# Xiugapurin/Etude

Measured on AMD Instinct MI355X. Metric: audio-sec/s transcribed + decoder tokens/s, 3-min clip batch, higher is better.
Workload: dtype f16

## Files before the change

### etude_amd/_lib.py

```python
from __future__ import annotations

import ctypes as C
import os
from pathlib import Path

import torch

LIB_PATH = Path(os.environ["ETD_LIB_PATH"]) if os.environ.get("ETD_LIB_PATH") else Path(__file__).resolve().parent / "libetude_hip.so"

c_int_p = C.POINTER(C.c_int)
c_i32_p = C.POINTER(C.c_int32)
c_i64_p = C.POINTER(C.c_int64)
c_f32_p = C.POINTER(C.c_float)


class _SizedCfg(C.Structure):

    def __init__(self, *a, **k):
        super().__init__(*a, **k)
        self.struct_bytes = C.sizeof(type(self))


class ExtCfg(_SizedCfg):
    _fields_ = [("struct_bytes", C.c_int)] + [(n, C.c_int) for n in ("n_margin", "n_frame", "n_bin", "cnn_channel", "cnn_kernel", "hid_dim", "pf_dim",
# ... 24 lines not shown
    _fields_ = [("struct_bytes", C.c_int), ("kernel", C.c_int), ("epi", C.c_int)] + [(n, C.c_int) for n in ("M", "N", "K", "ldx", "ldy")] + \
               [("X", C.c_void_p), ("x_elems", C.c_longlong), ("W", C.c_void_p), ("bias", C.c_void_p), ("x_bound", C.c_float),
                ("ln_g", C.c_void_p), ("ln_b", C.c_void_p), ("ln_eps", C.c_float), ("Y", C.c_void_p), ("y_elems", C.c_longlong),
                ("add", C.c_void_p), ("hin", C.c_void_p), ("hout", C.c_void_p), ("h_elems", C.c_longlong),
                ("pos", C.c_void_p), ("slot", C.c_void_p), ("active", C.c_void_p)] + [(n, C.c_int) for n in ("n_heads", "max_ctx", "n_slots", "rope_rows")] + \
               [("rope_cos", C.c_void_p), ("rope_sin", C.c_void_p), ("Q", C.c_void_p), ("q_elems", C.c_longlong), ("Kc", C.c_void_p), ("Vc", C.c_void_p), ("kv_elems", C.c_longlong)]


G3_KERNEL_AUTO, G3_KERNEL_TILE, G3_KERNEL_SMALL = 0, 1, 2
G3_EPI = {"bias": 0, "gelu": 1, "resid": 2, "logits": 3, "qkv": 4, "relu": 6}


class Job(C.Structure):
    _fields_ = [("x_ids", C.c_void_p), ("x_offsets", C.c_void_p), ("n_bars", C.c_int), ("attrs4", C.c_void_p), ("ready", C.c_void_p)]


class ScoreJob(C.Structure):
    _fields_ = [("x_ids", C.c_void_p), ("x_offsets", C.c_void_p), ("n_bars", C.c_int), ("attrs4", C.c_void_p),
                ("y_ids", C.c_void_p), ("y_offsets", C.c_void_p), ("n_y_bars", C.c_int)]


class SchedCfg(_SizedCfg):
    _fields_ = [("struct_bytes", C.c_int)] + [(n, C.c_int) for n in ("bar_bos_id", "bar_eos_id", "n_ctx_pairs", "max_position_embeddings", "max_output_tokens",
                                       "max_bar_token_limit")] + [("context_overlap_ratio", C.c_float)] + \
               [(n, C.c_int) for n in ("force_bar_tokens", "max_streams", "max_prefill_rows", "steps_per_poll")] + \
               [("temperature", C.c_float), ("top_p", C.c_float), ("seed", C.c_ulonglong), ("job_key_offset", C.c_int), ("job_key_stride", C.c_int)]


class TempoRegion(C.Structure):
    _fields_ = [("bpm", C.c_double), ("time_sig", C.c_int), ("start", C.c_double), ("downbeats", C.c_void_p), ("n_downbeats", C.c_int)]


class TokEvent(C.Structure):
    _fields_ = [("type", C.c_int32), ("value", C.c_int32)]


class Note(C.Structure):
    _fields_ = [("onset", C.c_double), ("offset", C.c_double), ("pitch", C.c_int32), ("velocity", C.c_int32)]


ABI_VERSION = 3

SIGNATURES = {
    "etd_version": (C.c_int, []),
    "etd_last_error": (C.c_char_p, []),
    "etd_build_id": (C.c_char_p, []),
    "etd_extractor_operand_type": (C.c_int, []),
    "etd_decoder_operand_type": (C.c_int, []),
    "etd_has_experiments": (C.c_int, []),
    "etd_prof_enable": (C.c_int, [C.c_int]),
    "etd_prof_reset": (C.c_int, []),
    "etd_prof_collect": (C.c_int, []),
    "etd_prof_count": (C.c_int, []),
    "etd_prof_entry": (C.c_int, [C.c_int, C.c_char_p, C.c_int, C.POINTER(C.c_double), C.POINTER(C.c_longlong),
                                 C.POINTER(C.c_double), C.POINTER(C.c_double)]),
    "etd_debug_boundary_cost": (C.c_int, [C.c_int, C.c_int, C.c_int, C.c_void_p, C.POINTER(C.c_double), C.POINTER(C.c_double)]),
    "etd_debug_linear": (C.c_int, [C.c_int, C.c_int, C.c_int, C.c_int, C.c_void_p, C.POINTER(C.c_double)]),
    "etd_debug_kernel_loop": (C.c_int, [C.c_int, C.c_int, C.c_void_p]),
    "etd_debug_g3_bounds": (C.c_int, [C.c_void_p, C.c_void_p, C.c_int, C.c_int, C.c_void_p, C.c_void_p, C.c_float, C.c_void_p, C.c_void_p]),
    "etd_debug_gemm3": (C.c_int, [C.c_void_p, C.c_int, C.c_int, C.c_void_p, C.c_void_p, C.c_int, C.c_float, C.c_int, C.c_void_p, C.c_void_p, C.c_void_p, C.c_void_p]),
    "etd_debug_gemm3_case": (C.c_int, [C.POINTER(G3Case), C.c_void_p]),
    "etd_debug_ln_rows_f32": (C.c_int, [C.c_void_p, C.c_int, C.c_int, C.c_void_p, C.c_void_p, C.c_void_p, C.c_void_p, C.c_float, C.c_void_p, C.c_void_p, C.c_void_p]),
    "etd_debug_g3_pack": (C.c_int, [C.c_void_p, C.c_int, C.c_int, C.c_void_p, C.c_longlong, C.POINTER(C.c_longlong), C.POINTER(C.c_int32)]),
    "etd_debug_attn3": (C.c_int, [C.c_void_p, C.c_void_p, C.c_void_p, C.c_void_p, C.c_int, C.c_int, C.c_int, C.c_int, C.c_float, C.c_float, C.c_float, C.c_int, C.c_void_p, C.c_void_p]),
    "etd_debug_empty_launch": (C.c_int, [C.c_int, C.c_int, C.c_int, C.c_void_p, C.c_void_p]),
    "etd_frontend_create": (C.c_int, [C.c_int, C.c_int, C.c_int, C.c_int, C.c_int, C.c_int, C.c_void_p, C.c_int, C.c_int,
                                      C.c_void_p, C.c_int, C.c_void_p, C.c_void_p, C.c_void_p, C.c_float, C.POINTER(C.c_void_p)]),
    "etd_frontend_destroy": (None, [C.c_void_p]),
    "etd_frontend_set_pad_mode": (C.c_int, [C.c_void_p, C.c_int]),
    "etd_rms_frames": (C.c_int, [C.c_void_p, C.c_longlong, C.c_int, C.c_int, C.c_void_p, C.c_longlong, C.c_void_p]),
    "etd_frontend_resampled_len": (C.c_longlong, [C.c_void_p, C.c_longlong]),
    "etd_frontend_num_frames": (C.c_longlong, [C.c_void_p, C.c_longlong]),
    "etd_frontend_run": (C.c_int, [C.c_void_p, C.c_void_p, C.c_int, C.c_longlong, C.c_void_p, C.c_void_p, C.c_longlong,
                                   C.POINTER(C.c_longlong), C.c_void_p]),
    "etd_extractor_create": (C.c_int, [C.POINTER(ExtCfg), C.POINTER(C.c_char_p), C.POINTER(C.c_void_p), c_i64_p, C.c_int,
                                       C.POINTER(C.c_void_p)]),
    "etd_extractor_destroy": (None, [C.c_void_p]),
    "etd_transcript": (C.c_int, [C.c_void_p, C.c_void_p, C.c_longlong] + [C.c_void_p] * 8 + [C.c_void_p]),
    "etd_transcript_windows": (C.c_int, [C.c_void_p, C.c_void_p, C.c_int] + [C.c_void_p] * 8 + [C.c_void_p]),
    "etd_extractor_debug_vel_logits": (C.c_int, [C.c_void_p, C.c_void_p]),
    "etd_extractor_debug_tap": (C.c_int, [C.c_void_p, C.c_int, C.c_void_p]),
    "etd_extractor_window_flops": (C.c_double, [C.c_void_p]),
    "etd_mpe2note": (C.c_int, [C.c_void_p, C.c_void_p, C.c_void_p, C.c_void_p, C.c_longlong, C.c_int, C.c_float, C.c_float,
                               C.c_float, C.c_int, C.c_int, C.c_int, C.POINTER(Note), C.c_longlong, C.POINTER(C.c_longlong)]),
    "etd_mpe2note_modes": (C.c_int, [C.c_void_p, C.c_void_p, C.c_void_p, C.c_void_p, C.c_longlong, C.c_int, C.c_float, C.c_float,
                                     C.c_float, C.c_int, C.c_int, C.c_int, C.c_int, C.c_int, C.POINTER(Note), C.c_longlong, C.POINTER(C.c_longlong)]),
    "etd_mpe2note_dev_create": (C.c_int, [C.c_int, C.POINTER(C.c_void_p)]),
    "etd_mpe2note_dev_destroy": (None, [C.c_void_p]),
    "etd_mpe2note_dev": (C.c_int, [C.c_void_p, C.c_void_p, C.c_void_p, C.c_void_p, C.c_void_p, C.c_longlong, C.c_float, C.c_float, C.c_float,
                                   C.c_int, C.c_int, C.c_int, C.POINTER(Note), C.c_longlong, C.POINTER(C.c_longlong), C.c_void_p]),
    "etd_mpe2note_dev_modes": (C.c_int, [C.c_void_p, C.c_void_p, C.c_void_p, C.c_void_p, C.c_void_p, C.c_longlong, C.c_float, C.c_float, C.c_float,
                                         C.c_int, C.c_int, C.c_int, C.c_int, C.c_int, C.POINTER(Note), C.c_longlong, C.POINTER(C.c_longlong), C.c_void_p]),
    "etd_tok_create": (C.c_int, [C.c_void_p, C.c_int, C.POINTER(C.c_void_p)]),
    "etd_tok_destroy": (None, [C.c_void_p]),
    "etd_tok_num_measures": (C.c_int, [C.c_void_p]),
    "etd_tok_measures": (C.c_int, [C.c_void_p, C.c_void_p, C.c_void_p, C.c_void_p, C.c_void_p]),
    "etd_tok_encode": (C.c_int, [C.c_void_p, C.c_void_p, C.c_longlong, C.c_int, C.c_void_p, C.c_longlong, C.POINTER(C.c_longlong)]),
    "etd_tok_split_bars": (C.c_int, [C.c_void_p, C.c_longlong, C.c_int, C.c_int, C.c_void_p, C.c_longlong, C.c_void_p, C.c_longlong,
                                     C.POINTER(C.c_longlong)]),
    "etd_tok_decode": (C.c_int, [C.c_void_p, C.c_void_p, C.c_longlong, C.c_void_p, C.c_longlong, C.c_void_p, C.c_longlong,
                                 C.POINTER(C.c_longlong)]),
    "etd_midi_write": (C.c_int, [C.c_void_p, C.c_longlong, C.c_char_p]),
    "etd_decoder_create": (C.c_int, [C.POINTER(DecCfg), C.POINTER(C.c_char_p), C.POINTER(C.c_void_p), c_i64_p, C.c_int,
                                     C.POINTER(C.c_void_p)]),
    "etd_decoder_destroy": (None, [C.c_void_p]),
    "etd_decoder_clone": (C.c_int, [C.c_void_p, C.POINTER(C.c_void_p)]),
    "etd_decoder_set_sampling": (C.c_int, [C.c_void_p, C.c_float, C.c_float, C.c_ulonglong, C.c_void_p]),
    "etd_decoder_set_keys": (C.c_int, [C.c_void_p, C.c_int, C.c_void_p, C.c_void_p]),
    "etd_decoder_begin_bar": (C.c_int, [C.c_void_p, C.c_int, C.c_void_p, C.c_void_p, C.c_void_p, C.c_int, C.c_void_p, C.c_int,
                                        C.c_int, C.c_void_p]),
    "etd_decoder_begin_bars": (C.c_int, [C.c_void_p, C.c_int] + [C.c_void_p] * 8 + [C.c_void_p]),
    "etd_decoder_step": (C.c_int, [C.c_void_p, C.c_void_p, C.c_int, C.c_int, C.c_void_p]),
    "etd_decoder_poll": (C.c_int, [C.c_void_p, C.c_void_p, C.c_int, C.c_void_p, C.c_void_p, C.c_void_p]),
    "etd_decoder_read_tokens": (C.c_int, [C.c_void_p, C.c_int, C.c_void_p, C.c_int, c_int_p, C.c_void_p]),
    "etd_decoder_read_many": (C.c_int, [C.c_void_p, C.c_int, C.c_void_p, C.c_void_p, C.c_int, C.c_void_p, C.c_void_p]),
    "etd_decoder_run_jobs": (C.c_int, [C.c_void_p, C.POINTER(SchedCfg), C.POINTER(Job), C.c_int, C.c_void_p, C.c_longlong, C.c_void_p,
                                       C.POINTER(C.c_longlong), C.c_void_p]),
    "etd_debug_assemble_prompt": (C.c_int, [C.POINTER(SchedCfg), C.c_int, C.c_void_p, C.c_void_p, C.c_void_p, C.c_void_p, C.c_void_p, C.c_void_p,
                                            C.c_int, C.c_void_p, C.c_void_p, C.c_void_p, C.c_void_p, C.c_int, c_int_p]),
    "etd_decoder_generate_bar": (C.c_int, [C.c_void_p, C.c_int, C.c_void_p, C.c_void_p, C.c_void_p, C.c_int, C.c_void_p,
                                           C.c_int, C.c_int, C.c_void_p, c_int_p, C.c_void_p]),
    "etd_decoder_prefill_logits": (C.c_int, [C.c_void_p, C.c_int, C.c_void_p, C.c_void_p, C.c_void_p, C.c_int, C.c_void_p,
                                             C.c_void_p]),
    "etd_decoder_score": (C.c_int, [C.c_void_p, C.c_int] + [C.c_void_p] * 11 + [C.c_void_p]),
    "etd_decoder_score_jobs": (C.c_int, [C.c_void_p, C.POINTER(SchedCfg), C.POINTER(ScoreJob), C.c_int, C.c_void_p, C.c_void_p, C.c_void_p, C.c_void_p]),
    "etd_debug_assemble_scored": (C.c_int, [C.POINTER(SchedCfg), C.c_int, C.c_void_p, C.c_void_p, C.c_void_p, C.c_void_p, C.c_void_p, C.c_void_p,
                                            C.c_int, C.c_void_p, C.c_int, C.c_void_p, C.c_void_p, C.c_void_p, C.c_void_p, C.c_void_p, C.c_int, c_int_p]),
    "etd_decoder_step_bytes": (C.c_double, [C.c_void_p, C.c_int, C.c_int]),
    "etd_decoder_stats": (C.c_int, [C.c_void_p, C.POINTER(C.c_double), C.c_int, C.c_void_p]),
    "etd_decoder_stats_reset": (C.c_int, [C.c_void_p, C.c_void_p]),
    "etd_decoder_stamp": (C.c_int, [C.c_void_p, C.c_int, C.c_int, C.c_void_p]),
    "etd_decoder_stamp_log": (C.c_int, [C.c_void_p, C.c_void_p, C.c_longlong, C.POINTER(C.c_longlong), C.c_void_p]),
    "etd_debug_decoder_force_pair": (C.c_int, [C.c_void_p, C.c_int]),
    "etd_debug_decoder_step_logits": (C.c_int, [C.c_void_p, C.c_int, C.c_void_p, C.c_int, C.c_void_p]),
    "etd_debug_decoder_checksum": (C.c_int, [C.c_void_p, C.POINTER(C.c_ulonglong), C.c_int, C.c_void_p]),
    "etd_debug_decoder_kv_rowsums": (C.c_int, [C.c_void_p, C.c_void_p, C.c_longlong, C.c_void_p]),
    "etd_debug_decoder_trace_begin": (C.c_int, [C.c_void_p, C.c_int, C.c_void_p]),
    "etd_debug_decoder_trace_slabs": (C.c_int, [C.c_void_p, C.c_void_p, C.c_longlong, C.c_int, C.c_void_p]),
    "etd_debug_decoder_trace_lanes": (C.c_int, [C.c_void_p, C.c_void_p, C.c_longlong, C.c_int, C.c_void_p]),
    "etd_debug_decoder_trace_q": (C.c_int, [C.c_void_p, C.c_void_p, C.c_longlong, C.c_int, C.c_void_p]),
    "etd_debug_decoder_peek_kv": (C.c_int, [C.c_void_p, C.c_int, C.c_int, C.c_int, C.c_int, C.c_void_p, C.c_void_p, C.c_void_p]),
    "etd_beat_create": (C.c_int, [C.POINTER(BeatCfg), C.POINTER(C.c_char_p), C.POINTER(C.c_void_p), c_i64_p, C.c_int, C.POINTER(C.c_void_p)]),
    "etd_beat_destroy": (None, [C.c_void_p]),
    "etd_beat_forward": (C.c_int, [C.c_void_p, C.c_void_p, C.c_int, c_i64_p, C.c_void_p, C.c_void_p, C.c_void_p]),
    "etd_beat_flops": (C.c_double, [C.c_void_p, C.c_longlong]),
    "etd_beat_debug_taps": (C.c_int, [C.c_void_p, C.c_void_p, C.c_void_p]),
    "etd_dbn_describe": (C.c_int, [C.POINTER(DbnCfg), C.c_int, C.c_void_p, C.c_int, c_int_p, c_int_p, c_int_p, C.c_void_p, C.c_void_p]),
    "etd_dbn_workspace_bytes": (C.c_longlong, [C.POINTER(DbnCfg), C.c_longlong, C.c_int]),
    "etd_dbn_create": (C.c_int, [C.POINTER(DbnCfg), C.POINTER(C.c_void_p)]),
    "etd_dbn_destroy": (None, [C.c_void_p]),
    "etd_dbn_track": (C.c_int, [C.c_void_p, C.c_void_p, C.c_int, C.c_int, c_i64_p, C.c_void_p, C.c_longlong, C.c_void_p, C.c_void_p, C.c_void_p, C.c_longlong,
                                C.c_void_p, C.c_void_p, C.POINTER(C.c_longlong), C.c_void_p]),
    "etd_dbn_debug_viterbi": (C.c_int, [C.c_void_p, C.c_int, C.c_void_p, C.c_longlong, C.c_void_p, C.POINTER(C.c_double)]),
    "etd_debug_decoder_trace_read": (C.c_int, [C.c_void_p, C.c_void_p, C.c_longlong, C.c_int, C.POINTER(C.c_int), C.c_void_p]),
}

_lib = None


class EtudeHipError(RuntimeError):
    pass


def lib() -> C.CDLL:
    global _lib
    if _lib is None:
        if not LIB_PATH.exists():
            raise EtudeHipError(f"{LIB_PATH} not found: build it with `python -m etude_amd.build` "
                                "(hipcc --offload-arch=gfx950); etude_amd has no CPU fallback")
        l = C.CDLL(str(LIB_PATH))
        for name, (res, args) in SIGNATURES.items():
            if os.environ.get("ETD_PARTIAL") and not hasattr(l, name):
                continue
            fn = getattr(l, name)
            fn.restype = res
            fn.argtypes = args
        if l.etd_version() != ABI_VERSION:
            raise EtudeHipError(f"{LIB_PATH} speaks ABI version {l.etd_version()}, this binding {ABI_VERSION}; rebuild with `python -m etude_amd.build`")
        if not os.environ.get("ETD_PARTIAL") and not os.environ.get("ETD_ALLOW_STALE_LIB"):
            from .build import src_hash
            have, want = (l.etd_build_id() or b"").decode(), src_hash()
            if have != want:
                raise EtudeHipError(f"{LIB_PATH} is stale: built from sources {have}, the tree is {want}; rebuild with `python -m etude_amd.build`")
        _lib = l
    return _lib


def check(rc: int, what: str = "") -> None:
    if rc != 0:
        msg = lib().etd_last_error()
        raise EtudeHipError(f"{what} failed (rc={rc}): {msg.decode() if msg else ''}")


def weights_arrays(state: dict):
    import numpy as np
    names = list(state.keys())
    arrs = [np.ascontiguousarray(np.asarray(state[k], dtype=np.float32)) for k in names]
    c_names = (C.c_char_p * len(names))(*[k.encode() for k in names])
    c_ptrs = (C.c_void_p * len(names))(*[a.ctypes.data for a in arrs])
    c_num = (C.c_int64 * len(names))(*[a.size for a in arrs])
    return c_names, c_ptrs, c_num, len(names), arrs


def prof_enable(on: bool) -> None:
    lib().etd_prof_enable(1 if on else 0)


def prof_reset() -> None:
    lib().etd_prof_reset()


def prof_report() -> dict:
    l = lib()
    l.etd_prof_collect()
    out = {}
    for i in range(l.etd_prof_count()):
        name = C.create_string_buffer(64)
        ms, n, fl, by = C.c_double(), C.c_longlong(), C.c_double(), C.c_double()
        check(l.etd_prof_entry(i, name, 64, C.byref(ms), C.byref(n), C.byref(fl), C.byref(by)), "etd_prof_entry")
        out[name.value.decode()] = dict(ms=ms.value, launches=n.value, flops=fl.value, bytes=by.value)
    return out
```

### etude_amd/csrc/api_dec.hip

```cpp
#include <algorithm>
#include <atomic>
#include <chrono>
#include <cmath>
#include <cstdlib>
#include <cstring>
#include <map>
#include <string>
#include <mutex>
#include <vector>

#include "../../include/etude_hip_debug.h"
#include "dec_kernels.h"
#include "gemm3.h"
#include "ext_kernels.h"
#include "dec_score.h"
#include "prof.h"

namespace {

inline uint16_t f2bf_h(float f) { return ETD_DEC_IS_F16 ? f32_to_f16_bits(f) : f32_to_bf16_bits(f); }

struct Lin { void* W = nullptr; float* b = nullptr; int N = 0, Npad = 0, K = 0;
             void* Wf = nullptr;
             G3Lin g3; };
// ... 177 lines not shown
  const Layer& w = d->layers[l];
  return launch_ln_rows(h, M, d->H, w.ln1g, w.ln1b, w.ln2g, w.ln2b, d->cfg.layer_norm_eps, d->X1b, d->X2b, st);
}
static int layer_dattn(etd_dec* d, int l, const DecRows& rows, int M, d16* Ob, int ldob, hipStream_t st) {
  DAttnArgs at = attn_args(d, l, rows, M); at.O = d->AO; at.Ob = Ob; at.ldob = ldob;
  if (rows.slot == d->row_slot) { attn_step_pairs(d, &at); attn_stamp(d, l, &at); }
  return launch_dattn(at, d->bf16w, st);
}
static int step_qkv_up(etd_dec* d, int l, const float* X, const DecRows& rows, int M, hipStream_t st) {
  DGemmArgs q = qkv_args(d, l, X, rows, M); q.Xb = d->X1b; q.Y = d->qkv_raw; q.ldy = 3 * d->H;
  DGemmArgs up = lin_args(d->layers[l].up, X, d->H, M); up.Xb = d->X2b; up.Y = d->M1; up.Yb = d->Xcat; up.ldy = d->I + d->H;
  return launch_dstep_qkv_up(q, up, st);
}
static int resid_ln(etd_dec* d, int l, int nslab, const float* hin, float* hout, int M, const NextLn& nx, hipStream_t st) {
  return launch_resid_ln_rows(d->Pk, nslab, d->layers[l].cat.b, nullptr, hin, hout, M, d->H, nx.g1, nx.b1, nx.g2, nx.b2, d->cfg.layer_norm_eps, nx.x1, nx.x2, st);
}
static int down_splitk(etd_dec* d, int l, const float* hin, float* hout, int M, const NextLn& nx, hipStream_t st) {
  DGemmArgs dn = lin_args(d->layers[l].cat, d->M1, d->I + d->H, M); dn.Xb = d->Xcat; dn.hin = hin; dn.hout = hout; dn.k_splits = DS_K_SPLITS; dn.Y = d->Pk; dn.ldy = d->H;
  ETD_TRY(launch_dgemm(dn, DEPI_PARTIAL, true, st));
  return resid_ln(d, l, DS_K_SPLITS, hin, hout, M, nx, st);
}
static int linear16(const Lin& w, const d16* X, int M, const DGemmArgs& dec, int epi, hipStream_t st) {
  LinArgs a = {};
  a.X = (const e16*)X; a.ldx = w.K; a.W = (const e16*)w.Wf;
  a.bias = w.b; a.M = M; a.N = w.N; a.K = w.K; a.vt_block = -1; a.dec = dec;
  return launch_linear_dec(a, epi, st);
}

static int gemm3_auto(const DGemmArgs& a, int epi, hipStream_t st) { return gemm3_s_takes(a, epi) ? launch_gemm3_s(a, epi, st) : launch_gemm3(a, epi, st); }
static int x3_last_rows(etd_dec* d, const LastOnly& lo, const float* hin, float* hout, hipStream_t st) {
  const int n = lo.n, l = d->L - 1, H = d->H; const Layer& w = d->layers[l];
  ETD_TRY(launch_gather_rows(hin, lo.idx, n, H, d->hlast, st)); ETD_TRY(launch_gather_rows(d->Q, lo.idx, n, H, d->t_q, st));
  DAttnArgs at = attn_args(d, l, lo.rows, n); at.Q = d->t_q; at.O = d->t_ao; at.bytes_hint = 0;
  ETD_TRY(launch_dattn(at, false, st));
  DGemmArgs de = lin_args(w.dense, d->t_ao, H, n); de.Y = d->t_do; de.ldy = H;
  ETD_TRY(launch_dgemm(de, DEPI_BIAS, false, st));
  DGemmArgs up = lin_args(w.up, d->hlast, H, n); up.Y = d->t_m1; up.ldy = d->I; up.ln_g = w.ln2g; up.ln_b = w.ln2b; up.ln_eps = d->cfg.layer_norm_eps;
  ETD_TRY(launch_dgemm(up, DEPI_GELU, false, st));
  DGemmArgs dn = lin_args(w.down, d->t_m1, d->I, n); dn.add = d->t_do; dn.hin = d->hlast; dn.hout = hout;
  return launch_dgemm(dn, DEPI_RESID, false, st);
}
static int x3_layer_rest(etd_dec* d, int l, const DecRows& rows, int M, const PrefillInfo* pf, const float* hin, float* hout, hipStream_t st) {
  const Layer& w = d->layers[l]; const int H = d->H;
  if (pf) {
    Attn3Args t = {};
    t.Q = d->Q; t.ldq = H; t.K = (const float*)kv_layer(d, d->Kc, l); t.V = (const float*)kv_layer(d, d->Vc, l); t.O = d->AO; t.ldo = H; t.n_seq = pf->n; t.n_heads = d->nh;
    t.seq_row0 = pf->seq_row0; t.seq_len = pf->seq_len; t.row_slot = rows.slot; t.slot_stride = d->slot_stride; t.max_ctx = d->ctx; t.max_len = pf->max_len;
    t.scale = 0.125f; t.q_log2 = w.q_log2; t.k_log2 = w.k_log2; t.v_log2 = w.v_log2; t.flops_hint = pf->attn_flops;
    ETD_TRY(launch_attn3(t, st));
  } else {
    DAttnArgs at = attn_args(d, l, rows, M);
    at.O = d->AO; attn_stamp(d, l, &at);
    if (rows.slot == d->row_slot) attn_step_pairs(d, &at);
    ETD_TRY(launch_dattn(at, false, st));
  }
  DGemmArgs de = lin_args(w.dense, d->AO, H, M); de.Y = d->DO; de.ldy = H;
  ETD_TRY(gemm3_auto(de, DEPI_BIAS, st));
  DGemmArgs up = lin_args(w.up, d->X2f, H, M); up.Y = d->M1; up.ldy = d->I;
  ETD_TRY(gemm3_auto(up, DEPI_GELU, st));
  DGemmArgs dn = lin_args(w.down, d->M1, d->I, M); dn.add = d->DO; dn.hin = hin; dn.hout = hout;
  return gemm3_auto(dn, DEPI_RESID, st);
}
static int forward_x3(etd_dec* d, int M, const DecRows& rows, const PrefillInfo* pf, const LastOnly* lo, hipStream_t st, float** hfinal, bool* compact) {
  const bool tail = lo && pf && lo->n >= 1 && lo->n < G3_MIN_ROWS && lo->n <= d->S;
  float* hin = d->h; float* hout = d->h2;
  for (int l = 0; l < d->L; ++l) {
    const Layer& w = d->layers[l];
    ETD_TRY(launch_ln_rows_f32(hin, M, d->H, w.ln1g, w.ln1b, w.ln2g, w.ln2b, d->cfg.layer_norm_eps, d->X1f, d->X2f, st));
    ETD_TRY(gemm3_auto(qkv_args(d, l, d->X1f, rows, M), DEPI_QKV, st));
    ETD_TRY(tail && l == d->L - 1 ? x3_last_rows(d, *lo, hin, hout, st) : x3_layer_rest(d, l, rows, M, pf, hin, hout, st));
    std::swap(hin, hout);
  }
  *hfinal = hin; if (tail) *compact = true;
  return ETD_OK;
}

static int forward_plain(etd_dec* d, int M, const DecRows& rows, bool act16, hipStream_t st, float** hfinal) {
  float* hin = d->h; float* hout = d->h2; const float eps = d->cfg.layer_norm_eps;
  for (int l = 0; l < d->L; ++l) {
    const Layer& w = d->layers[l];
    if (act16) ETD_TRY(ln_rows16(d, l, hin, M, st));
    DGemmArgs q = qkv_args(d, l, hin, rows, M); q.Y = d->qkv_raw; q.ldy = 3 * d->H;
    if (act16) q.Xb = d->X1b; else { q.ln_g = w.ln1g; q.ln_b = w.ln1b; q.ln_eps = eps; }
    ETD_TRY(launch_dgemm(q, DEPI_QKV, d->bf16w, st));
    ETD_TRY(layer_dattn(d, l, rows, M, act16 ? d->AOb : nullptr, 0, st));
    DGemmArgs de = lin_args(w.dense, d->AO, d->H, M); de.Y = d->DO; de.ldy = d->H; if (act16) de.Xb = d->AOb;
    ETD_TRY(launch_dgemm(de, DEPI_BIAS, d->bf16w, st));
    DGemmArgs up = lin_args(w.up, hin, d->H, M); up.Y = d->M1; up.ldy = d->I;
    if (act16) { up.Xb = d->X2b; up.Yb = d->M1b; } else { up.ln_g = w.ln2g; up.ln_b = w.ln2b; up.ln_eps = eps; }
    ETD_TRY(launch_dgemm(up, DEPI_GELU, d->bf16w, st));
    DGemmArgs dn = lin_args(w.down, d->M1, d->I, M); dn.add = d->DO; dn.hin = hin; dn.hout = hout; if (act16) dn.Xb = d->M1b;
    ETD_TRY(launch_dgemm(dn, DEPI_RESID, d->bf16w, st));
    std::swap(hin, hout);
  }
  *hfinal = hin;
  return ETD_OK;
}

static int trace_qkv_up(etd_dec* d, int l, int M, hipStream_t st) {
  if (!d->trace) return ETD_OK;
  ETD_TRY(trace_rows(d, d->Q, d->H, d->H, 1, 0, M, l * ETD_TRACE_LAYER * M, st));
  if (l == 0) HIP_TRY(hipMemcpyAsync(d->trace_q, d->Q, (size_t)M * d->H * 4, hipMemcpyDeviceToDevice, st));
  ETD_TRY(trace_rows(d, d->Xcat, (d->I + d->H) / 2, d->I / 2, 1, 0, M, l * ETD_TRACE_LAYER * M + M, st));
  if (d->nh == 8) {
    hipLaunchKernelGGL(k_trace_kv, dim3(M, 8), dim3(64), 0, st, (const unsigned*)kv_layer(d, d->Kc, l), (const unsigned*)kv_layer(d, d->Vc, l), d->slot_stride / 2, d->ctx,
                       d->row_slot, d->row_pos, M, d->trace, d->trace_step, d->trace_cap, trace_wps(d, M), l * ETD_TRACE_LAYER * M + 17 * M);
    HIP_TRY(hipGetLastError());
  }
  return ETD_OK;
}
static int skinny_attn_down(etd_dec* d, int l, const DecRows& rows, int M, const float* hin, float* hout, hipStream_t st) {
  const Layer& w = d->layers[l]; const NextLn nx = next_ln(d, l);
  const int ksd = d->I / 512;
  DAttnArgs at = attn_args(d, l, rows, M);
  attn_step_pairs(d, &at); attn_stamp(d, l, &at); at.pair = d->step_pair ? 1 : 0;
  at.dense_w = (const d16*)w.dense_hw; at.dense_out = d->Pk + (size_t)ksd * M * d->H; at.dbg = (d->trace && l == 0) ? d->trace_dbg : nullptr;
  DGemmArgs dn = lin_args(w.cat, nullptr, d->I + d->H, M); dn.Xb = d->Xcat; dn.k_splits = ksd; dn.Y = d->Pk; dn.ldy = d->H;
  if (rowfin_on() && ksd + d->nh == 12 && M <= DS_STEP_MAX_ROWS) {
    DRowFin fin = {};
    fin.cnt = d->row_cnt + (size_t)l * DS_STEP_MAX_ROWS; fin.target = d->nh + 16 * ksd; fin.P = d->Pk; fin.nslab = 12;
    fin.bias = w.cat.b; fin.hin = hin; fin.hout = hout; fin.eps = d->cfg.layer_norm_eps;
    fin.g1 = nx.g1; fin.b1 = nx.b1; fin.g2 = nx.g2; fin.b2 = nx.b2; fin.x1 = nx.x1; fin.x2 = nx.x2;
    return launch_dstep_attn_down(at, dn, &fin, st);
  }
  ETD_TRY(launch_dstep_attn_down(at, dn, nullptr, st));
  if (d->trace && ksd + d->nh == 12) ETD_TRY(trace_rows(d, d->Pk, d->H, d->H, 12, (long long)M * d->H, M, l * ETD_TRACE_LAYER * M + 2 * M, st));
  if (d->trace && l == 0 && ksd + d->nh == 12) HIP_TRY(hipMemcpyAsync(d->trace_pk, d->Pk, (size_t)12 * M * d->H * 4, hipMemcpyDeviceToDevice, st));
  ETD_TRY(resid_ln(d, l, ksd + d->nh, hin, hout, M, nx, st));
  if (d->trace) {
    ETD_TRY(trace_rows(d, hout, d->H, d->H, 1, 0, M, l * ETD_TRACE_LAYER * M + 14 * M, st));
    if (nx.x1) {
      ETD_TRY(trace_rows(d, d->X1b, d->H / 2, d->H / 2, 1, 0, M, l * ETD_TRACE_LAYER * M + 15 * M, st));
      ETD_TRY(trace_rows(d, d->X2b, d->H / 2, d->H / 2, 1, 0, M, l * ETD_TRACE_LAYER * M + 16 * M, st));
    }
  }
  return ETD_OK;
}
static int forward_skinny16(etd_dec* d, int M, const DecRows& rows, bool ln0_done, hipStream_t st, float** hfinal) {
  const bool attn_down = rows.slot == d->row_slot && d->H == 512 && d->nh == 8 && d->I % 512 == 0 && d->I / 512 + d->nh <= 12 && d->layers[0].dense_hw &&
                         d->ctx >= 256 && !getenv("ETD_NO_ATTN_DOWN");
  float* hin = d->h; float* hout = d->h2;
  if (!ln0_done) ETD_TRY(ln_rows16(d, 0, hin, M, st));
  for (int l = 0; l < d->L; ++l) {
    ETD_TRY(step_qkv_up(d, l, hin, rows, M, st));
    ETD_TRY(trace_qkv_up(d, l, M, st));
    if (attn_down) ETD_TRY(skinny_attn_down(d, l, rows, M, hin, hout, st));
    else { ETD_TRY(layer_dattn(d, l, rows, M, d->Xcat + d->I, d->I + d->H, st)); ETD_TRY(down_splitk(d, l, hin, hout, M, next_ln(d, l), st)); }
    std::swap(hin, hout);
  }
  *hfinal = hin;
  return ETD_OK;
}

static int prefill16_qkv(etd_dec* d, int l, const float* hin, const DecRows& rows, int M, bool mfma_attn, hipStream_t st) {
  const Layer& w = d->layers[l];
  DGemmArgs q = qkv_args(d, l, hin, rows, M); q.Xb = d->X1b; q.Y = d->qkv_raw; q.ldy = 3 * d->H;
  if (mfma_attn) q.Qb = d->Qb;
  static const bool pqkv_on = !getenv("ETD_NO_PQKV");
  if (!(mfma_attn && pqkv_on && M >= 49152 && d->H == 512 && d->nh == 8 && w.qkv.N == 1536)) return linear16(w.qkv, d->X1b, M, q, DEPI_QKV, st);
  PQkvArgs pa = {};
  pa.X = d->X1b; pa.ldx = d->H; pa.Wf = (const d16*)w.qkv.Wf; pa.bias = w.qkv.b; pa.M = M; pa.N = w.qkv.N; pa.rows = rows;
  pa.rope_cos = d->rope_cos; pa.rope_sin = d->rope_sin; pa.Qb = d->Qb; pa.Kc = (d16*)q.Kc; pa.Vc = (d16*)q.Vc; pa.slot_stride = d->slot_stride; pa.max_ctx = d->ctx; pa.n_heads = d->nh;
  return launch_pqkv(pa, st);
}
static int prefill16_layer_rest(etd_dec* d, int l, const DecRows& rows, int M, const PrefillInfo* pf, bool fmlp, const float* hin, float* hout, hipStream_t st) {
  const Layer& w = d->layers[l];
  if (pf) {
    PAttnArgs t = {};
    t.Q = d->Qb; t.ldq = d->H; t.Kc = (const d16*)kv_layer(d, d->Kc, l); t.Vc = (const d16*)kv_layer(d, d->Vc, l); t.slot_stride = d->slot_stride; t.max_ctx = d->ctx; t.n_heads = d->nh;
    t.O = d->Xcat + d->I; t.ldo = d->I + d->H; t.seq_row0 = pf->seq_row0; t.seq_len = pf->seq_len; t.row_slot = rows.slot;
    t.n_seq = pf->n; t.max_len = pf->max_len; t.scale_log2e = 0.125f * 1.4426950408889634f; t.flops_hint = pf->attn_flops;
    ETD_TRY(launch_pattn(t, st));
  } else ETD_TRY(layer_dattn(d, l, rows, M, d->Xcat + d->I, d->I + d->H, st));
  if (fmlp) {
    const NextLn nx = next_ln(d, l); DMlpArgs ma = {};
    ma.X2 = d->X2b; ma.AO = d->Xcat + d->I; ma.ldao = d->I + d->H; ma.hin = hin; ma.hout = hout; ma.Wm = (const d16*)w.mlp_frag;
    ma.b_up = w.up.b; ma.b_cat = w.cat.b; ma.eps = d->cfg.layer_norm_eps; ma.M = M;
    ma.g1 = nx.g1; ma.b1 = nx.b1; ma.g2 = nx.g2; ma.b2 = nx.b2; ma.nx1 = nx.x1; ma.nx2 = nx.x2;
    return launch_dmlp_fused(ma, st);
  }
  DGemmArgs up = {}; up.Yb = d->Xcat; up.ldy = d->I + d->H;
  ETD_TRY(linear16(w.up, d->X2b, M, up, DEPI_GELU, st));
  DGemmArgs dn = {}; dn.N = d->H; dn.hin = hin; dn.hout = hout;
  return linear16(w.cat, d->Xcat, M, dn, DEPI_RESID, st);
}
static int prefill16_last_rows(etd_dec* d, const LastOnly& lo, const float* hin, float* hout, hipStream_t st) {
  const int n = lo.n, l = d->L - 1;
  ETD_TRY(launch_gather_rows(hin, lo.idx, n, d->H, d->hlast, st));
  ETD_TRY(ln_rows16(d, l, d->hlast, n, st));
  ETD_TRY(step_qkv_up(d, l, d->hlast, lo.rows, n, st));
  DAttnArgs at = attn_args(d, l, lo.rows, n); at.O = d->AO; at.Ob = d->Xcat + d->I; at.ldob = d->I + d->H; at.bytes_hint = 0;
  ETD_TRY(launch_dattn(at, d->bf16w, st));
  return down_splitk(d, l, d->hlast, hout, n, NextLn{}, st);
}
static int forward_prefill16(etd_dec* d, int M, const DecRows& rows, const PrefillInfo* pf, const LastOnly* lo, hipStream_t st, float** hfinal, bool* compact) {
  const bool fmlp = d->layers[0].mlp_frag && d->H == 512 && d->I == 2048 && fused_pmlp_on();
  const bool tail = lo && pf && lo->n > 1 && lo->n <= DS_STEP_MAX_ROWS && step_shape(d) && !getenv("ETD_NO_LAST_ONLY");
  float* hin = d->h; float* hout = d->h2;
  for (int l = 0; l < d->L; ++l) {
    if (l == 0 || !fmlp) ETD_TRY(ln_rows16(d, l, hin, M, st));
    ETD_TRY(prefill16_qkv(d, l, hin, rows, M, pf != nullptr, st));
    ETD_TRY(tail && l == d->L - 1 ? prefill16_last_rows(d, *lo, hin, hout, st) : prefill16_layer_rest(d, l, rows, M, pf, fmlp, hin, hout, st));
    std::swap(hin, hout);
  }
  *hfinal = hin; if (tail) *compact = true;
  return ETD_OK;
}

static int forward_rows(etd_dec* d, int M, const DecRows& rows, const PrefillInfo* pf, const LastOnly* lo, hipStream_t st, float** hfinal, bool* compact) {
  if (compact) *compact = false; else lo = nullptr;
  const Layer& w0 = d->layers[0];
  if (!d->bf16w && M >= G3_MIN_ROWS && d->X1f && w0.qkv.g3.Wp && w0.down.g3.Wp && g3_enabled()) return forward_x3(d, M, rows, pf, lo, st, hfinal, compact);
  const bool act16 = d->bf16w && M > 1;
  if (act16 && M > DS_MAX_ROWS && w0.qkv.Wf && w0.up.Wf && w0.cat.Wf) return forward_prefill16(d, M, rows, pf, lo, st, hfinal, compact);
  if (act16 && ksplit_fits(d)) return forward_skinny16(d, M, rows, false, st, hfinal);
  return forward_plain(d, M, rows, act16, st, hfinal);
}

int head_logits(etd_dec* d, const float* X, int n, float* logits, hipStream_t st) {
  const bool g3 = !d->bf16w && n >= G3_MIN_ROWS && d->X1f && d->head.g3.Wp && g3_enabled();
  if (g3) ETD_TRY(launch_ln_rows_f32(X, n, d->H, d->lnfg, d->lnfb, nullptr, nullptr, d->cfg.layer_norm_eps, d->X1f, nullptr, st));
  DGemmArgs lm = lin_args(d->head, g3 ? d->X1f : X, d->H, n);
  lm.bias = nullptr; lm.Y = logits; lm.ldy = d->V;
  if (g3) return launch_gemm3(lm, DEPI_LOGITS, st);
  lm.ln_g = d->lnfg; lm.ln_b = d->lnfb; lm.ln_eps = d->cfg.layer_norm_eps;
  return launch_dgemm(lm, DEPI_LOGITS, d->bf16w, st);
}

int check_slot(etd_dec* d, int slot) {
  if (!d || slot < 0 || slot >= d->S) ETD_FAIL(ETD_EINVAL, "decoder: bad slot %d", slot);
  return ETD_OK;
}

__global__ void k_init_slots(const int* __restrict__ init, int n, int* tgt_attrs, int* cur_tok, int* len, int* done, int* n_out, int* eos, int* limit) {
  const int i = blockIdx.x * blockDim.x + threadIdx.x;
  if (i >= n) return;
  const int* p = init + i * 7;
  const int s = p[0];
  tgt_attrs[4 * s] = p[1]; tgt_attrs[4 * s + 1] = p[2]; tgt_attrs[4 * s + 2] = p[3]; tgt_attrs[4 * s + 3] = p[4];
  cur_tok[s] = 0; len[s] = 0; done[s] = 0; n_out[s] = 0; eos[s] = p[5]; limit[s] = p[6];
}

__global__ __launch_bounds__(128) void k_slot_proj(const int* __restrict__ init, const float* __restrict__ attr_tab, int n_bins, int H, float* proj) {
  const int* p = init + blockIdx.x * 7;
  const int s = p[0];
  for (int k = threadIdx.x * 4; k < H; k += 128 * 4) {
    f32x4 t[4];
#pragma unroll
    for (int a = 0; a < 4; ++a) t[a] = *reinterpret_cast<const f32x4*>(attr_tab + (long long)(a * n_bins + p[1 + a]) * H + k);
    f32x4 o;
#pragma unroll
    for (int c = 0; c < 4; ++c) o[c] = ((t[0][c] + t[1][c]) + t[2][c]) + t[3][c];
    *reinterpret_cast<f32x4*>(proj + (long long)s * H + k) = o;
  }
}

struct Staged { int Mtot; const int *ids, *cls, *attrs, *row_slot, *row_pos, *row_active, *last_idx, *last_slot, *last_pos, *last_active, *init, *row_seq, *seq_row0, *seq_len; };

int stage_and_forward(etd_dec* d, int n, const int32_t* slots, const int32_t* T, const int32_t* ids, const int32_t* cls,
                      const int32_t* attrs4, const int32_t* init7 , Staged* sg, float** hfinal, hipStream_t st, bool* last_only = nullptr) {
  if (!d || n < 1 || n > d->S || !slots || !T || !ids || !cls || !attrs4) ETD_FAIL(ETD_EINVAL, "prefill: bad arguments");
  long long Mtot = 0;
  std::vector<char> seen((size_t)d->S, 0);
  for (int i = 0; i < n; ++i) {
    ETD_TRY(check_slot(d, slots[i]));
    if (T[i] <= 0 || T[i] > d->ctx) ETD_FAIL(ETD_EINVAL, "prefill: prompt %d has T=%d (max_ctx=%d)", i, T[i], d->ctx);
    if (seen[slots[i]]) ETD_FAIL(ETD_EINVAL, "prefill: slot %d listed twice", slots[i]);
    seen[slots[i]] = 1;
    Mtot += T[i];
  }
  if (Mtot > d->Mcap) ETD_FAIL(ETD_EINVAL, "prefill: %lld prompt rows exceed max_prefill_rows=%d", Mtot, d->Mcap);
  const int M = (int)Mtot;
  for (int i = 0; i < M; ++i) {
    if (ids[i] < 0 || ids[i] >= d->V || cls[i] < 0 || cls[i] >= d->cfg.num_classes) ETD_FAIL(ETD_EINVAL, "prefill: token/class id out of range at row %d", i);
    for (int k = 0; k < 4; ++k) if (attrs4[(size_t)k * M + i] < 0 || attrs4[(size_t)k * M + i] >= d->cfg.num_attribute_bins) ETD_FAIL(ETD_EINVAL, "prefill: attribute bin out of range at row %d", i);
  }
  const size_t sv_ints = (size_t)10 * M + 13 * n;
  int* svp;
  const bool pinned = d->pin_stage && sv_ints <= d->pin_stage_ints;
  if (pinned) {
    HIP_TRY(hipEventSynchronize(d->pin_stage_evt));
    svp = d->pin_stage;
  } else {
    d->stage.resize(sv_ints);
    svp = d->stage.data();
  }
  memcpy(svp, ids, (size_t)M * 4);
  memcpy(svp + M, cls, (size_t)M * 4);
  memcpy(svp + 2 * (size_t)M, attrs4, (size_t)4 * M * 4);
  int* rs = svp + 6 * (size_t)M; int* rp = rs + M; int* ra = rp + M;
  int* li = ra + M; int* ls = li + n; int* lp = ls + n; int* la = lp + n; int* in7 = la + n;
  int* rq = in7 + 7 * n; int* sr0 = rq + M; int* sln = sr0 + n;
  int row = 0, max_len = 0; double kvb = 0, aflops = 0;
  for (int i = 0; i < n; ++i) {
    sr0[i] = row; sln[i] = T[i]; if (T[i] > max_len) max_len = T[i];
    aflops += 0.5 * 256.0 * d->nh * (double)T[i] * T[i];
    for (int t = 0; t < T[i]; ++t, ++row) { rs[row] = slots[i]; rp[row] = t; ra[row] = 1; rq[row] = i; }
    li[i] = row - 1; ls[i] = slots[i]; lp[i] = T[i] - 1; la[i] = 1;
    d->host_len[slots[i]] = T[i];
    kvb += (double)T[i] * d->nh * 64 * (2.0 * (d->bf16w ? 2 : 4) + 4 + 4);
  }
  if (init7) memcpy(in7, init7, (size_t)7 * n * 4); else memset(in7, 0, (size_t)7 * n * 4);
  d->attn_bytes_hint = kvb;
  HIP_TRY(hipMemcpyAsync(d->ids, svp, sv_ints * 4, hipMemcpyHostToDevice, st));
  if (pinned) HIP_TRY(hipEventRecord(d->pin_stage_evt, st));
  d->host_n_out_valid = false;
  const int* b = d->ids;
  *sg = Staged{M, b, b + M, b + 2 * (size_t)M, b + 6 * (size_t)M, b + 7 * (size_t)M, b + 8 * (size_t)M, b + 9 * (size_t)M, b + 9 * (size_t)M + n,
               b + 9 * (size_t)M + 2 * n, b + 9 * (size_t)M + 3 * n, b + 9 * (size_t)M + 4 * n,
               b + 9 * (size_t)M + 11 * n, b + 10 * (size_t)M + 11 * n, b + 10 * (size_t)M + 12 * n};
  if (init7) {
    hipLaunchKernelGGL(k_init_slots, dim3((n + 63) / 64), dim3(64), 0, st, sg->init, n, d->tgt_attrs, d->cur_tok, d->len, d->done, d->n_out, d->eos, d->limit);
    HIP_TRY(hipGetLastError());
    hipLaunchKernelGGL(k_slot_proj, dim3(n), dim3(128), 0, st, sg->init, d->attr_tab, d->cfg.num_attribute_bins, d->H, d->tgt_proj);
    HIP_TRY(hipGetLastError());
  }
  DEmbedArgs e = {};
  e.ids = sg->ids; e.cls = sg->cls; e.attrs = sg->attrs; e.M = M; e.H = d->H; e.n_bins = d->cfg.num_attribute_bins;
  e.word = d->word; e.cls_emb = d->cls_emb; e.attr_tab = d->attr_tab; e.h = d->h;
  e.rows = DecRows{sg->row_slot, sg->row_pos, sg->row_active, sg->row_seq};
  ETD_TRY(launch_dembed(e, st));
  PrefillInfo pf{n, sg->seq_row0, sg->seq_len, max_len, aflops};
  const bool can_mfma_attn = (d->bf16w ? d->Qb != nullptr : d->X1f != nullptr) && !ETD_XENV("ETD_NO_MFMA_PREFILL_ATTN");
  LastOnly lo{n, sg->last_idx, DecRows{sg->last_slot, sg->last_pos, sg->last_active}};
  return forward_rows(d, M, e.rows, can_mfma_attn ? &pf : nullptr, &lo, st, hfinal, last_only);
}

int alloc_workspaces(etd_dec* d) {
  const int H = d->H;
  DevPool& P = d->pool;
  d->slot_stride = (long long)d->nh * d->ctx * 64;
  d->layer_stride = d->slot_stride * d->S;
  const size_t kv_elems = (size_t)d->layer_stride * d->L;
  if (d->bf16w) { uint16_t *k, *v; ETD_TRY(P.alloc(&k, kv_elems, true)); ETD_TRY(P.alloc(&v, kv_elems, true)); d->Kc = k; d->Vc = v; }
  else { float *k, *v; ETD_TRY(P.alloc(&k, kv_elems, true)); ETD_TRY(P.alloc(&v, kv_elems, true)); d->Kc = k; d->Vc = v; }
  const size_t M = d->Mcap;
  const size_t Mf = d->bf16w ? (size_t)(d->S > 1 ? d->S : 1) : M;
  ETD_TRY(P.alloc(&d->h, M * H)); ETD_TRY(P.alloc(&d->h2, M * H));
  ETD_TRY(P.alloc(&d->Q, M * H)); ETD_TRY(P.alloc(&d->AO, M * H)); ETD_TRY(P.alloc(&d->DO, M * H));
  ETD_TRY(P.alloc(&d->M1, Mf * d->I)); ETD_TRY(P.alloc(&d->logits, (size_t)d->Mmax * d->V));
  ETD_TRY(P.alloc(&d->qkv_raw, (size_t)3 * H)); ETD_TRY(P.alloc(&d->hlast, (size_t)d->S * H));
  if (d->bf16w) {
    ETD_TRY(P.alloc(&d->X1b, M * H)); ETD_TRY(P.alloc(&d->X2b, M * H)); ETD_TRY(P.alloc(&d->AOb, M * H));
    ETD_TRY(P.alloc(&d->M1b, M * d->I));
    ETD_TRY(P.alloc(&d->Pk, (size_t)12 * DS_STEP_MAX_ROWS * H));
    ETD_TRY(P.alloc(&d->row_cnt, (size_t)d->L * DS_STEP_MAX_ROWS, true));
    ETD_TRY(P.alloc(&d->Xcat, M * (d->I + H)));
    ETD_TRY(P.alloc(&d->Qb, M * H));
  }
  if (!d->bf16w) {
    ETD_TRY(P.alloc(&d->X1f, M * H)); ETD_TRY(P.alloc(&d->X2f, M * H));
    const size_t Sr = d->S > 1 ? d->S : 1;
    ETD_TRY(P.alloc(&d->t_q, Sr * H)); ETD_TRY(P.alloc(&d->t_ao, Sr * H)); ETD_TRY(P.alloc(&d->t_do, Sr * H)); ETD_TRY(P.alloc(&d->t_m1, Sr * d->I));
  }
// ... 658 lines not shown
  const bool full = logits_dev != nullptr;
  std::vector<int32_t> slots(S), a4c, up;
  for (int i = 0; i < S; ++i) slots[i] = i;
  long long r0 = 0;
  for (int i0 = 0; i0 < n;) {
    int k = 0; long long Mc = 0;
    while (i0 + k < n && k < S && (k == 0 || Mc + T[i0 + k] <= rowcap)) Mc += T[i0 + k++];
    const int mc = (int)Mc;
    a4c.resize((size_t)4 * mc);
    for (int a = 0; a < 4; ++a) memcpy(a4c.data() + (size_t)a * mc, attrs4 + a * M + r0, (size_t)mc * 4);
    up.assign(labels + r0, labels + r0 + mc);
    for (int r = 0; r < mc; ++r) if (full || labels[r0 + r] != ETD_IGNORE_LABEL) up.push_back(r);
    const int nl = (int)up.size() - mc;
    const int nblk = (nl + hb - 1) / hb;
    up.resize((size_t)mc + (size_t)nblk * hb, 0);
    HIP_TRY(hipMemcpyAsync(lab_dev, up.data(), (size_t)mc * 4, hipMemcpyHostToDevice, st));
    if (nblk) HIP_TRY(hipMemcpyAsync(idx_dev, up.data() + mc, (size_t)nblk * hb * 4, hipMemcpyHostToDevice, st));
    up.clear();
    for (int i = 0, row = 0; i < k; ++i) { up.push_back(row); row += T[i0 + i]; }
    up.insert(up.end(), T + i0, T + i0 + k);
    HIP_TRY(hipMemcpyAsync(r0_dev, up.data(), (size_t)k * 4, hipMemcpyHostToDevice, st));
    HIP_TRY(hipMemcpyAsync(len_dev, up.data() + k, (size_t)k * 4, hipMemcpyHostToDevice, st));
    if (row_lp || row_argmax) {
      HIP_TRY(hipMemsetAsync(lp_dev, 0, (size_t)mc * 4, st));
      HIP_TRY(hipMemsetAsync(am_dev, 0xff, (size_t)mc * 4, st));
    }
    Staged sg; float* hf = nullptr;
    ETD_TRY(stage_and_forward(d, k, slots.data(), T + i0, ids + r0, cls + r0, a4c.data(), nullptr, &sg, &hf, st));
    for (int b = 0; b < nblk; ++b) {
      const int nb = std::min(hb, nl - b * hb);
      ETD_TRY(launch_gather_rows(hf, idx_dev + (size_t)b * hb, hb, d->H, d->sc_x, st));
      ETD_TRY(head_logits(d, d->sc_x, hb, d->logits, st));
      ETD_TRY(launch_row_logprob(d->logits, d->V, d->V, nb, idx_dev + (size_t)b * hb, lab_dev, lp_dev, lse_dev, am_dev, st));
      if (full) HIP_TRY(hipMemcpyAsync(logits_dev + (size_t)(r0 + (long long)b * hb) * d->V, d->logits, (size_t)nb * d->V * 4, hipMemcpyDeviceToDevice, st));
    }
    ETD_TRY(launch_seq_reduce(r0_dev, len_dev, k, lab_dev, lp_dev, am_dev, d->sc_d, tok_dev, hit_dev, st));
    HIP_TRY(hipMemcpyAsync(seq_logprob + i0, d->sc_d, (size_t)k * sizeof(double), hipMemcpyDeviceToHost, st));
    HIP_TRY(hipMemcpyAsync(seq_tokens + i0, tok_dev, (size_t)k * 4, hipMemcpyDeviceToHost, st));
    HIP_TRY(hipMemcpyAsync(seq_hits + i0, hit_dev, (size_t)k * 4, hipMemcpyDeviceToHost, st));
    if (row_lp) HIP_TRY(hipMemcpyAsync(row_lp + r0, lp_dev, (size_t)mc * 4, hipMemcpyDeviceToHost, st));
    if (row_argmax) HIP_TRY(hipMemcpyAsync(row_argmax + r0, am_dev, (size_t)mc * 4, hipMemcpyDeviceToHost, st));
    HIP_TRY(hipStreamSynchronize(st));
    i0 += k; r0 += mc;
  }
  return ETD_OK;
}

__global__ void k_sum_words(const unsigned* __restrict__ p, long long n, unsigned long long* out) {
  unsigned long long s = 0;
  for (long long i = blockIdx.x * (long long)blockDim.x + threadIdx.x; i < n; i += (long long)gridDim.x * blockDim.x) s += (unsigned long long)p[i] * (unsigned long long)((i & 1023) + 1);
  for (int o = 32; o > 0; o >>= 1) s += __shfl_xor(s, o, 64);
  if ((threadIdx.x & 63) == 0) atomicAdd(out, s);
}
extern "C" int etd_debug_decoder_checksum(etd_dec* d, unsigned long long* out, int cap, void* stream) {
  hipStream_t st = (hipStream_t)stream;
  if (!d || !out || cap < 1) ETD_FAIL(ETD_EINVAL, "decoder_checksum: bad arguments");
  const size_t first = d->weights_owner ? 0 : d->n_weight_allocs;
  const size_t n = d->pool.ptrs.size() - first;
  unsigned long long* acc = nullptr;
  HIP_TRY(hipMalloc(&acc, 8 * (n + 1)));
  HIP_TRY(hipMemsetAsync(acc, 0, 8 * (n + 1), st));
  for (size_t i = 0; i < n; ++i)
    hipLaunchKernelGGL(k_sum_words, dim3(1024), dim3(256), 0, st, (const unsigned*)d->pool.ptrs[first + i], (long long)(d->pool.bytes[first + i] / 4), acc + 1 + i);
  std::vector<unsigned long long> h(n + 1);
  HIP_TRY(hipMemcpyAsync(h.data(), acc, 8 * (n + 1), hipMemcpyDeviceToHost, st));
  HIP_TRY(hipStreamSynchronize(st));
  (void)hipFree(acc);
  for (size_t i = 1; i <= n; ++i) h[0] += h[i];
  for (int i = 0; i < cap; ++i) out[i] = (size_t)i <= n ? h[i] : 0ull;
  return ETD_OK;
}

__global__ void k_kv_rowsums(const unsigned* __restrict__ K, const unsigned* __restrict__ V, int L, int S, int nh, int ctx, unsigned* out) {
  const long long i = blockIdx.x * (long long)blockDim.x + threadIdx.x;
  if (i >= (long long)L * S * ctx) return;
  const int pos = (int)(i % ctx), slot = (int)((i / ctx) % S), l = (int)(i / ((long long)ctx * S));
  unsigned s = 0;
  for (int hd = 0; hd < nh; ++hd) {
    const long long w0 = ((((long long)l * S + slot) * nh + hd) * ctx + pos) * 32;
    for (int w = 0; w < 32; ++w) s += K[w0 + w] * (unsigned)(w + 1 + 64 * hd) + V[w0 + w] * (unsigned)(w + 33 + 64 * hd);
  }
  out[i] = s;
}
extern "C" int etd_debug_decoder_kv_rowsums(etd_dec* d, unsigned* out_host, long long cap, void* stream) {
  hipStream_t st = (hipStream_t)stream;
  if (!d || !out_host || !d->bf16w) ETD_FAIL(ETD_EINVAL, "kv_rowsums: d16 handles only");
  const long long n = (long long)d->L * d->S * d->ctx;
  if (cap < n) ETD_FAIL(ETD_ENOMEM, "kv_rowsums: need room for %lld words", n);
  unsigned* dev = nullptr;
  HIP_TRY(hipMalloc(&dev, n * 4));
  hipLaunchKernelGGL(k_kv_rowsums, dim3((unsigned)((n + 255) / 256)), dim3(256), 0, st, (const unsigned*)d->Kc, (const unsigned*)d->Vc, d->L, d->S, d->nh, d->ctx, dev);
  HIP_TRY(hipMemcpyAsync(out_host, dev, n * 4, hipMemcpyDeviceToHost, st));
  HIP_TRY(hipStreamSynchronize(st));
  (void)hipFree(dev);
  return ETD_OK;
}

extern "C" int etd_debug_decoder_trace_begin(etd_dec* d, int cap_steps, void* stream) {
  hipStream_t st = (hipStream_t)stream;
  if (!d || cap_steps < 1 || !d->bf16w) ETD_FAIL(ETD_EINVAL, "trace_begin: bad args");
  HIP_TRY(hipStreamSynchronize(st));
  for (auto& kv : d->graphs) (void)hipGraphExecDestroy(kv.second);
  d->graphs.clear();
  if (d->trace) { (void)hipFree(d->trace); d->trace = nullptr; }
  if (d->trace_step) { (void)hipFree(d->trace_step); d->trace_step = nullptr; }
  if (d->trace_pk) { (void)hipFree(d->trace_pk); d->trace_pk = nullptr; }
  if (d->trace_q) { (void)hipFree(d->trace_q); d->trace_q = nullptr; }
  HIP_TRY(hipMalloc(&d->trace_pk, (size_t)12 * d->S * d->H * 4));
  HIP_TRY(hipMalloc(&d->trace_q, (size_t)d->S * d->H * 4));
  if (!d->trace_dbg) HIP_TRY(hipMalloc(&d->trace_dbg, (size_t)d->nh * d->S * 256 * 8 * 4));
  const size_t bytes = (size_t)cap_steps * trace_wps(d, d->S) * 4;
  HIP_TRY(hipMalloc(&d->trace, bytes));
  HIP_TRY(hipMalloc(&d->trace_step, 4));
  HIP_TRY(hipMemsetAsync(d->trace, 0, bytes, st));
  HIP_TRY(hipMemsetAsync(d->trace_step, 0, 4, st));
  HIP_TRY(hipStreamSynchronize(st));
  d->trace_cap = cap_steps;
  return ETD_OK;
}
extern "C" int etd_debug_decoder_trace_slabs(etd_dec* d, float* out_host, long long cap_floats, int n_active, void* stream) {
  hipStream_t st = (hipStream_t)stream;
  if (!d || !d->trace_pk || !out_host || n_active < 1 || n_active > d->S) ETD_FAIL(ETD_EINVAL, "trace_slabs: bad args");
  const long long n = 12LL * n_active * d->H;
  if (cap_floats < n) ETD_FAIL(ETD_ENOMEM, "trace_slabs: need room for %lld floats", n);
  HIP_TRY(hipMemcpyAsync(out_host, d->trace_pk, (size_t)n * 4, hipMemcpyDeviceToHost, st));
  HIP_TRY(hipStreamSynchronize(st));
  return ETD_OK;
}
extern "C" int etd_debug_decoder_trace_lanes(etd_dec* d, float* out_host, long long cap_floats, int n_active, void* stream) {
  hipStream_t st = (hipStream_t)stream;
  const long long n = (long long)(d ? d->nh : 0) * n_active * 256 * 8;
  if (!d || !d->trace_dbg || !out_host || n_active < 1 || n_active > d->S || cap_floats < n) ETD_FAIL(ETD_EINVAL, "trace_lanes: bad args");
  HIP_TRY(hipMemcpyAsync(out_host, d->trace_dbg, (size_t)n * 4, hipMemcpyDeviceToHost, st));
  HIP_TRY(hipStreamSynchronize(st));
  return ETD_OK;
}
extern "C" int etd_debug_decoder_trace_q(etd_dec* d, float* out_host, long long cap_floats, int n_active, void* stream) {
  hipStream_t st = (hipStream_t)stream;
  if (!d || !d->trace_q || !out_host || n_active < 1 || n_active > d->S || cap_floats < (long long)n_active * d->H) ETD_FAIL(ETD_EINVAL, "trace_q: bad args");
  HIP_TRY(hipMemcpyAsync(out_host, d->trace_q, (size_t)n_active * d->H * 4, hipMemcpyDeviceToHost, st));
  HIP_TRY(hipStreamSynchronize(st));
  return ETD_OK;
}
extern "C" int etd_debug_decoder_peek_kv(etd_dec* d, int layer, int slot, int head, int n_pos, unsigned short* k_out, unsigned short* v_out, void* stream) {
  hipStream_t st = (hipStream_t)stream;
  if (!d || !d->bf16w || layer < 0 || layer >= d->L || slot < 0 || slot >= d->S || head < 0 || head >= d->nh || n_pos < 1 || n_pos > d->ctx || !k_out || !v_out)
    ETD_FAIL(ETD_EINVAL, "peek_kv: bad args");
  const size_t off = ((size_t)layer * d->layer_stride + (size_t)slot * d->slot_stride + (size_t)head * d->ctx * 64) * 2;
  HIP_TRY(hipMemcpyAsync(k_out, (const char*)d->Kc + off, (size_t)n_pos * 128, hipMemcpyDeviceToHost, st));
  HIP_TRY(hipMemcpyAsync(v_out, (const char*)d->Vc + off, (size_t)n_pos * 128, hipMemcpyDeviceToHost, st));
  HIP_TRY(hipStreamSynchronize(st));
  return ETD_OK;
}
extern "C" int etd_debug_decoder_trace_read(etd_dec* d, unsigned* out_host, long long cap_words, int n_active, int* steps_done, void* stream) {
  hipStream_t st = (hipStream_t)stream;
  if (!d || !d->trace || !out_host || !steps_done || n_active < 1 || n_active > d->S) ETD_FAIL(ETD_EINVAL, "trace_read: bad args");
  const long long n = (long long)d->trace_cap * trace_wps(d, n_active);
  if (cap_words < n) ETD_FAIL(ETD_ENOMEM, "trace_read: need room for %lld words", n);
  HIP_TRY(hipMemcpyAsync(out_host, d->trace, (size_t)n * 4, hipMemcpyDeviceToHost, st));
  HIP_TRY(hipMemcpyAsync(steps_done, d->trace_step, 4, hipMemcpyDeviceToHost, st));
  HIP_TRY(hipStreamSynchronize(st));
  return ETD_OK;
}

extern "C" double etd_decoder_step_bytes(const etd_dec* d, int n_streams, int ctx) {
  const double esz = d->bf16w ? 2.0 : 4.0;
  double w = 0;
  for (const Layer& l : d->layers) w += ((double)l.qkv.N * l.qkv.K + (double)l.dense.N * l.dense.K + (double)l.up.N * l.up.K + (double)l.down.N * l.down.K) * esz;
  w += (double)d->V * d->H * esz;
  const double kv = (double)n_streams * 2.0 * d->L * (double)(ctx + 1) * d->H * esz;
  return w + kv;
}
```

### etude_amd/csrc/dec_kernels.h

```cpp
#pragma once
#include "common.h"

#ifdef ETD_DEC_BF16
typedef bf16 d16; typedef bf16x8 d16x8; typedef bf16x4 d16x4; typedef bf16x2 d16x2;
#define ETD_MFMA16_DEC "v_mfma_f32_32x32x16_bf16"
#define ETD_DEC_IS_F16 0
#ifdef __HIPCC__
__device__ __forceinline__ d16x4 pack4d(float a, float b, float c, float d) { return pack4(a, b, c, d); }
#endif
#else
typedef f16 d16; typedef f16x8 d16x8; typedef f16x4 d16x4; typedef f16x2 d16x2;
#define ETD_MFMA16_DEC "v_mfma_f32_32x32x16_f16"
#define ETD_DEC_IS_F16 1
#ifdef __HIPCC__
__device__ __forceinline__ d16x4 pack4d(float a, float b, float c, float d) { return pack4h(a, b, c, d); }
#endif
#endif

#define DS_MAX_ROWS 512
#define DS_STEP_MAX_ROWS 2048

struct DecRows {
  const int* slot;
  const int* pos;
  const int* active;
  const int* seq;
};

struct DSampleCfg { float inv_temp; float top_p; unsigned long long seed; };

#define ETD_STAMP_HDR (8 + 2 * 64)
#define ETD_STAMP_LOGCAP 131072

enum { DEPI_BIAS = 0, DEPI_GELU = 1, DEPI_RESID = 2, DEPI_LOGITS = 3, DEPI_QKV = 4, DEPI_PARTIAL = 5, DEPI_RELU = 6  };

struct DGemmArgs {
  const float* X; int ldx;
  const void* W;
  const void* Wf;
  const float* bias;
  int M, N, K;
  int Npad;
  const float* ln_g; const float* ln_b; float ln_eps;
  float* Y; int ldy;
  d16* Yb;
  int k_splits;
  const d16* Xb;
  const float* add; const float* hin; float* hout;
  DecRows rows;
  const float* rope_cos; const float* rope_sin;
  int rot_half;
  float* Q;
  void* Kc; void* Vc;
  long long slot_stride;
  int max_ctx, n_heads;
  d16* Qb;
  const void* Wp; int w_log2;
  int x_log2;
};
int launch_dgemm(const DGemmArgs& a, int epi, bool w_bf16, hipStream_t st);
int launch_dstep_qkv_up(const DGemmArgs& q, const DGemmArgs& up, hipStream_t st);

struct DHeadArgs {
  const float* hfin; int M, H, V, Vpad;
  const float* lnf_g; const float* lnf_b; float eps;
  const d16* Whead;
  int* row_slot; int* row_pos; int* row_active; int* row_sp;
  int* cur_tok; int* len; int* done; int* n_out; int* out_tok; int out_cap; const int* eos; const int* limit;
  const int* tgt_attrs; const float* tgt_proj ; int tgt_cls; int n_bins;
  const float* word; const float* cls_emb; const float* attr_tab;
  const float* g1; const float* b1; const float* g2; const float* b2;
  float* h; d16* x1; d16* x2;
  const DSampleCfg* samp; const unsigned long long* rng_key;
  float* logits_dbg;
};
int launch_dstep_head(const DHeadArgs& a, hipStream_t st);

struct DAttnArgs {
  const float* Q;
  const void* Kc; const void* Vc; long long slot_stride; int max_ctx, n_heads;
  DecRows rows; int M;
  const int* row_sp;
  int identity;
  int pair;
  float* O;
  d16* Ob; int ldob;
  float scale;
  double bytes_hint;
  const d16* dense_w;
  float* dense_out;
  float* dbg;
  unsigned long long* stamp;
  int stamp_par;
};
int launch_dattn(const DAttnArgs& a, bool kv_bf16, hipStream_t st);
struct DRowFin {
  int* cnt; int target;
  const float* P; int nslab;
  const float* bias; const float* hin; float* hout;
  const float* g1; const float* b1; const float* g2; const float* b2; float eps;
  d16* x1; d16* x2;
};
int launch_dstep_attn_down(const DAttnArgs& a, const DGemmArgs& down, const DRowFin* fin, hipStream_t st);

struct PAttnArgs {
  const d16* Q; int ldq;
  const d16* Kc; const d16* Vc;
  long long slot_stride; int max_ctx, n_heads;
  d16* O; int ldo;
  const int* seq_row0; const int* seq_len; const int* row_slot;
  int n_seq, max_len;
  float scale_log2e;
  double flops_hint;
};
int launch_pattn(const PAttnArgs& a, hipStream_t st);

struct PQkvArgs {
  const d16* X; int ldx;
  const d16* Wf;
  const float* bias;
  int M, N;
  DecRows rows;
  const float* rope_cos; const float* rope_sin;
  d16* Qb;
  d16* Kc; d16* Vc; long long slot_stride; int max_ctx, n_heads;
};
int launch_pqkv(const PQkvArgs& a, hipStream_t st);

int launch_ln_rows(const float* h, int M, int H, const float* g1, const float* b1, const float* g2, const float* b2, float eps,
                   d16* x1, d16* x2, hipStream_t st);
int launch_resid_ln_rows(const float* P, int k_splits, const float* bias, const float* add, const float* hin, float* hout, int M, int H,
                         const float* g1, const float* b1, const float* g2, const float* b2, float eps, d16* x1, d16* x2, hipStream_t st);
int launch_gather_rows(const float* src, const int* idx, int n, int H, float* out, hipStream_t st);

#define DMLP_NCHUNK 73
#define DMLP_STREAM_ELEMS (DMLP_NCHUNK * 32 * 1024)
struct DMlpArgs {
  const d16* X2;
  const d16* AO; int ldao;
  const float* hin; float* hout;
  const d16* Wm;
  const float* b_up;
  const float* b_cat;
  const float* g1; const float* b1; const float* g2; const float* b2; float eps;
  d16* nx1; d16* nx2;
  int M;
};
int launch_dmlp_fused(const DMlpArgs& a, hipStream_t st);
void pack_dmlp_weights(const uint16_t* Wup_bf16 , const uint16_t* Wcat_bf16 , uint16_t* dst );

struct DEmbedArgs {
  const int* ids; const int* cls; const int* attrs;
  const int* cur_tok; const int* tgt_attrs;
  int tgt_cls;
  DecRows rows; int M, H, n_bins;
  const int* slots; const int* len; const int* done;
  int* row_slot_out; int* row_pos_out; int* row_active_out; int* row_sp_out;
  const float* word; const float* cls_emb; const float* attr_tab;
  float* h;
};
int launch_dembed(const DEmbedArgs& a, hipStream_t st);

struct DArgmaxArgs {
  const float* logits; int ldl; int V; int M;
  DecRows rows;
  int* cur_tok; int* len; int* done; int* n_out; int* out_tok; int out_cap; const int* eos; const int* limit;
  int set_len_from_pos;
  const DSampleCfg* samp; const unsigned long long* rng_key;
};
int launch_dargmax(const DArgmaxArgs& a, hipStream_t st);
```

### etude_amd/csrc/dec_kernels.hip

```cpp
#include "dec_kernels.h"
#include "prof.h"

#define DLD32 36
#define DLD16 72

#include "dec_epilogue.h"

#ifdef ETD_STEP_STAMP
__device__ long long* g_ss_buf;
__device__ unsigned long long g_ss_cap;
__device__ unsigned long long g_ss_cnt;
#define SS_DECL() long long ss_t[6] = {0, 0, 0, 0, 0, 0}
#define SS(i) do { __builtin_amdgcn_sched_barrier(0); ss_t[i] = (long long)__builtin_amdgcn_s_memrealtime(); __builtin_amdgcn_sched_barrier(0); } while (0)
#define SS_LANDED() asm volatile("s_waitcnt vmcnt(0)" ::: "memory")
#define SS_FLUSH(kid, role) do { if (threadIdx.x == 0 && g_ss_buf) { const unsigned long long i_ = atomicAdd(&g_ss_cnt, 1ull); if (i_ < g_ss_cap) { long long* o_ = g_ss_buf + i_ * 8;          \
      o_[0] = (long long)(kid) | ((long long)(role) << 8) | ((long long)blockIdx.x << 16); o_[1] = ss_t[0]; o_[2] = ss_t[1]; o_[3] = ss_t[2]; o_[4] = ss_t[3]; o_[5] = ss_t[4]; o_[6] = ss_t[5];   \
      o_[7] = (long long)__builtin_amdgcn_s_getreg((20 << 0) | (0 << 6) | (3 << 11)); } } } while (0)
extern "C" int etd_debug_step_stamps(long long* dev_buf, unsigned long long cap_records, unsigned long long* count_out) {
  HIP_TRY(hipDeviceSynchronize());
  if (count_out) HIP_TRY(hipMemcpyFromSymbol(count_out, HIP_SYMBOL(g_ss_cnt), 8));
  const unsigned long long zero = 0;
  HIP_TRY(hipMemcpyToSymbol(HIP_SYMBOL(g_ss_cnt), &zero, 8));
  HIP_TRY(hipMemcpyToSymbol(HIP_SYMBOL(g_ss_buf), &dev_buf, 8));
  HIP_TRY(hipMemcpyToSymbol(HIP_SYMBOL(g_ss_cap), &cap_records, 8));
// ... 376 lines not shown

#define QMT_PITCH 144
__global__ __launch_bounds__(256) __attribute__((amdgpu_waves_per_eu(2, 2))) void k_dstep_qkv_up_mt(int p_M, int split128, int p_ftiles128, const d16* p_Wfq, const d16* p_Wfu, const d16* p_Xq, const d16* p_Xu,
                                                         int p_ldxq, int p_ldxu, DGemmArgs q, DGemmArgs up) {
  __shared__ __attribute__((aligned(16))) unsigned char smem[2 * 128 * QMT_PITCH];
  const int tid = threadIdx.x, lane = tid & 63, wave = tid >> 6, r = lane & 31, h = lane >> 5, fh = wave & 1, rh = wave >> 1;
  const int M = p_M, K = 512;
  const int RT = (M + 127) / 128, bid = blockIdx.x, ft = ((bid >> 3) / RT) * 8 + (bid & 7);
  if (ft >= p_ftiles128) return;
  const bool isq = ft < split128;
  const int mwg = ((bid >> 3) % RT) * 128, m0 = mwg + rh * 64, n0 = (isq ? ft : ft - split128) * 128 + fh * 64;
  const d16* wfrag = (isq ? p_Wfq : p_Wfu) + ((long long)(n0 / 32) * (K / 16) * 64 + lane) * 8;
  const d16* xbase = isq ? p_Xq : p_Xu;
  const int ldx = isq ? p_ldxq : p_ldxu;
  const d16* xsrc[4]; int xdst[4];
#pragma unroll
  for (int i = 0; i < 4; ++i) {
    const int pce = tid + 256 * i, row = pce >> 3, c = pce & 7;
    int gmr = mwg + row; gmr = gmr < M ? gmr : M - 1;
    xsrc[i] = xbase + (long long)gmr * ldx + c * 8;
    xdst[i] = row * QMT_PITCH + c * 16;
  }
  int gm[2];
#pragma unroll
  for (int t = 0; t < 2; ++t) { gm[t] = m0 + 32 * t + r; gm[t] = gm[t] < M ? gm[t] : M - 1; }
  int pos[2], slot[2], act[2];
#pragma unroll
  for (int t = 0; t < 2; ++t) { pos[t] = q.rows.pos[gm[t]]; slot[t] = q.rows.slot[gm[t]]; act[t] = q.rows.active[gm[t]]; }
  f32x4 bq[2][4];
#pragma unroll
  for (int f = 0; f < 2; ++f) {
    const float* bp = (isq ? q.bias : up.bias) + n0 + 32 * f + 4 * h;
#pragma unroll
    for (int q4 = 0; q4 < 4; ++q4) bq[f][q4] = *reinterpret_cast<const f32x4*>(bp + 8 * q4);
  }
  f32x16 acc[2][2], accA[2][2];
#pragma unroll
  for (int f = 0; f < 2; ++f)
#pragma unroll
    for (int t = 0; t < 2; ++t)
#pragma unroll
      for (int i = 0; i < 16; ++i) acc[f][t][i] = 0.f;
  u32x4 xr[4];
  d16x8 wf[2][4][2];
  auto xrequest = [&](int c) {
#pragma unroll
    for (int i = 0; i < 4; ++i) xr[i] = *reinterpret_cast<const u32x4*>(xsrc[i] + c * 64);
  };
  auto wrequest = [&](int c, int b) {
#pragma unroll
    for (int s4 = 0; s4 < 4; ++s4)
#pragma unroll
      for (int f = 0; f < 2; ++f) wf[b][s4][f] = *reinterpret_cast<const d16x8*>(wfrag + (long long)((f * 32 + c * 4 + s4) * 64) * 8);
  };
  xrequest(0); wrequest(0, 0);
#pragma unroll
  for (int half = 0; half < 2; ++half) {
#pragma unroll
    for (int cc = 0; cc < 4; ++cc) {
      const int c = half * 4 + cc, b = c & 1;
      unsigned char* xb = smem + b * (128 * QMT_PITCH);
#pragma unroll
      for (int i = 0; i < 4; ++i) *reinterpret_cast<u32x4*>(xb + xdst[i]) = xr[i];
      __syncthreads();
      if (c + 1 < 8) { xrequest(c + 1); wrequest(c + 1, b ^ 1); }
#pragma unroll
      for (int s4 = 0; s4 < 4; ++s4) {
        d16x8 xf[2];
#pragma unroll
        for (int t = 0; t < 2; ++t) xf[t] = *reinterpret_cast<const d16x8*>(xb + (rh * 64 + 32 * t + r) * QMT_PITCH + s4 * 32 + h * 16);
#pragma unroll
        for (int f = 0; f < 2; ++f)
#pragma unroll
          for (int t = 0; t < 2; ++t) acc[f][t] = mfma32(wf[b][s4][f], xf[t], acc[f][t]);
      }
    }
    if (half == 0) {
#pragma unroll
      for (int f = 0; f < 2; ++f)
#pragma unroll
        for (int t = 0; t < 2; ++t) {
          accA[f][t] = acc[f][t];
#pragma unroll
          for (int i = 0; i < 16; ++i) acc[f][t][i] = 0.f;
        }
    }
  }
  __syncthreads();
  unsigned char* sw = smem + wave * (64 * QMT_PITCH);
  const int head = n0 / 192, part = (n0 - head * 192) >> 6;
  const int er = lane >> 3, ec = lane & 7;
  float vv[2][2][16];
#pragma unroll
  for (int f = 0; f < 2; ++f) {
    const bool rope = isq && part < 2 && f == 0;
#pragma unroll
    for (int t = 0; t < 2; ++t) {
      f32x16 a2;
#pragma unroll
      for (int i = 0; i < 16; ++i) a2[i] = accA[f][t][i] + acc[f][t][i];
      f32x4 rc = {1.f, 1.f, 1.f, 1.f}, rs = {0.f, 0.f, 0.f, 0.f};
      if (rope) {
        rc = *reinterpret_cast<const f32x4*>(q.rope_cos + (long long)pos[t] * 8 + 4 * h);
        rs = *reinterpret_cast<const f32x4*>(q.rope_sin + (long long)pos[t] * 8 + 4 * h);
      }
      qkv_up_tile_values(a2, bq[f], isq, rope, rc, rs, vv[f][t]);
    }
  }
  if (!isq || part != 0) {
#pragma unroll
    for (int f = 0; f < 2; ++f)
#pragma unroll
      for (int t = 0; t < 2; ++t)
#pragma unroll
        for (int q4 = 0; q4 < 4; ++q4)
          *reinterpret_cast<d16x4*>(sw + (32 * t + r) * 144 + (32 * f + 8 * q4 + 4 * h) * 2) = pack4d(vv[f][t][4 * q4], vv[f][t][4 * q4 + 1], vv[f][t][4 * q4 + 2], vv[f][t][4 * q4 + 3]);
    __builtin_amdgcn_wave_barrier();
#pragma unroll
    for (int it = 0; it < 8; ++it) {
      const int row = it * 8 + er, m = m0 + row;
      const u32x4 val = *reinterpret_cast<const u32x4*>(sw + row * 144 + ec * 16);
      const int rl = row & 31, tt = row >> 5;
      const int ps = __shfl(tt ? pos[1] : pos[0], rl, 64), sl = __shfl(tt ? slot[1] : slot[0], rl, 64), ac = __shfl(tt ? act[1] : act[0], rl, 64);
      if (m >= M) continue;
      if (!isq) {
        if (n0 + ec * 8 < up.N) *reinterpret_cast<u32x4*>(up.Yb + (long long)m * up.ldy + n0 + ec * 8) = val;
      } else {
        if (ac && ps < q.max_ctx)
          *reinterpret_cast<u32x4*>(reinterpret_cast<d16*>(part == 1 ? q.Kc : q.Vc) + (long long)sl * q.slot_stride + ((long long)head * q.max_ctx + ps) * 64 + ec * 8) = val;
      }
    }
  } else {
#pragma unroll
    for (int f = 0; f < 2; ++f) {
#pragma unroll
      for (int t = 0; t < 2; ++t)
#pragma unroll
        for (int q4 = 0; q4 < 4; ++q4) {
          const f32x4 o = {vv[f][t][4 * q4], vv[f][t][4 * q4 + 1], vv[f][t][4 * q4 + 2], vv[f][t][4 * q4 + 3]};
          *reinterpret_cast<f32x4*>(sw + (32 * t + r) * 144 + (8 * q4 + 4 * h) * 4) = o;
        }
      __builtin_amdgcn_wave_barrier();
#pragma unroll
      for (int it = 0; it < 8; ++it) {
        const int row = it * 8 + er, m = m0 + row;
        const u32x4 val = *reinterpret_cast<const u32x4*>(sw + row * 144 + ec * 16);
        if (m < M) *reinterpret_cast<u32x4*>(q.Q + (long long)m * (q.n_heads * 64) + head * 64 + 32 * f + ec * 4) = val;
      }
      __builtin_amdgcn_wave_barrier();
    }
  }
}

int launch_dstep_qkv_up(const DGemmArgs& q, const DGemmArgs& up, hipStream_t st) {
  if (q.M != up.M || q.K != up.K || q.M < 1 || q.M > DS_STEP_MAX_ROWS || !q.Xb || !up.Xb || !up.Yb || q.K != 512 || q.Npad % 32 || up.Npad % 32 ||
      q.rot_half != 8 || q.N % 192 || q.Qb || !q.Q || !q.bias || !up.bias || up.N % 4)
    ETD_FAIL(ETD_EINVAL, "dstep_qkv_up: bad arguments");
  ProfScope ps("k_dstep_qkv_up", st, 2.0 * q.M * (q.N + up.N) * q.K, (double)(q.Npad + up.Npad) * q.K * 2);
  const int split = q.Npad / 32;
  const int ftiles = split + up.Npad / 32;
  static const bool mt_on = !(ETD_XENV("ETD_QKV_MT") && atoi(ETD_XENV("ETD_QKV_MT")) == 0);
  static const int mt_min = ETD_XENV("ETD_QKV_MT_MIN") ? atoi(ETD_XENV("ETD_QKV_MT_MIN")) : 256;
  if (mt_on && q.M >= mt_min && q.Npad % 128 == 0 && up.Npad % 128 == 0 && q.Wf && up.Wf) {
    const int split128 = q.Npad / 128, ft128 = split128 + up.Npad / 128, RT128 = (q.M + 127) / 128;
    hipLaunchKernelGGL(k_dstep_qkv_up_mt, dim3((unsigned)(((ft128 + 7) / 8) * 8 * RT128)), dim3(256), 0, st, q.M, split128, ft128, (const d16*)q.Wf, (const d16*)up.Wf, q.Xb, up.Xb, q.ldx, up.ldx, q, up);
    HIP_TRY(hipGetLastError());
    return ETD_OK;
  }
  static const int rpt_env = ETD_XENV("ETD_QKV_RPT") ? atoi(ETD_XENV("ETD_QKV_RPT")) : 0;
  const int rpt = rpt_env > 0 ? rpt_env : (q.M > DS_MAX_ROWS ? 4 : 1);
  const int RT = (q.M + 31) / 32, RG = (RT + rpt - 1) / rpt;
  hipLaunchKernelGGL(k_dstep_qkv_up, dim3((unsigned)(((ftiles + 7) / 8) * 8 * RG)), dim3(64 * DS_WAVES), 0, st, q.M, q.K, split, ftiles, q.W, up.W, q.Xb, up.Xb, q.ldx, up.ldx, rpt, q, up);
  HIP_TRY(hipGetLastError());
  return ETD_OK;
}

__device__ __forceinline__ unsigned long long mix64(unsigned long long z) {
  z += 0x9e3779b97f4a7c15ull;
  z = (z ^ (z >> 30)) * 0xbf58476d1ce4e5b9ull;
  z = (z ^ (z >> 27)) * 0x94d049bb133111ebull;
  return z ^ (z >> 31);
}
__device__ __forceinline__ int wave_argmax(const float* lg, int V, int lane) {
  float best = -INFINITY; int bi = 0x7fffffff;
  for (int v = lane; v < V; v += 64) {
    const float x = lg[v];
    if (x > best || (x == best && v < bi)) { best = x; bi = v; }
  }
#define ETD_AMAX_STAGE(O) { const float ob = lane_xor<O>(best); const int oi = lane_xor<O>(bi); \
    const bool take = (ob > best) | ((ob == best) & (oi < bi)); best = take ? ob : best; bi = take ? oi : bi; }
  ETD_AMAX_STAGE(32) ETD_AMAX_STAGE(16) ETD_AMAX_STAGE(8) ETD_AMAX_STAGE(4) ETD_AMAX_STAGE(2) ETD_AMAX_STAGE(1)
#undef ETD_AMAX_STAGE
  return bi;
}
__device__ __forceinline__ void wave_argmax4(const float* lg, int ld, int V, int lane, int (&out)[4]) {
  float best[4]; int bi[4];
#pragma unroll
  for (int j = 0; j < 4; ++j) { best[j] = -INFINITY; bi[j] = 0x7fffffff; }
#pragma unroll
  for (int it = 0; it < 4; ++it) {
    const int v = lane + 64 * it;
    float x[4];
#pragma unroll
    for (int j = 0; j < 4; ++j) x[j] = lg[j * ld + (v < V ? v : 0)];
#pragma unroll
    for (int j = 0; j < 4; ++j) {
      const bool take = (v < V) & ((x[j] > best[j]) | ((x[j] == best[j]) & (v < bi[j])));
      best[j] = take ? x[j] : best[j]; bi[j] = take ? v : bi[j];
    }
  }
#define ETD_AMAX_STAGE(O) _Pragma("unroll") for (int j = 0; j < 4; ++j) { const float ob = lane_xor<O>(best[j]); const int oi = lane_xor<O>(bi[j]); \
    const bool take = (ob > best[j]) | ((ob == best[j]) & (oi < bi[j])); best[j] = take ? ob : best[j]; bi[j] = take ? oi : bi[j]; }
  ETD_AMAX_STAGE(32) ETD_AMAX_STAGE(16) ETD_AMAX_STAGE(8) ETD_AMAX_STAGE(4) ETD_AMAX_STAGE(2) ETD_AMAX_STAGE(1)
#undef ETD_AMAX_STAGE
#pragma unroll
  for (int j = 0; j < 4; ++j) out[j] = bi[j];
}
__device__ __attribute__((noinline)) int wave_sample(const float* lg, int V, int lane, float inv_temp, float top_p, unsigned long long seed, unsigned long long key,
                           unsigned ctr, float* sp, float* ss, int* si) {
  float mx = -INFINITY;
  for (int v = lane; v < V; v += 64) mx = fmaxf(mx, lg[v] * inv_temp);
  mx = wave_max(mx);
  float sum = 0.f;
  for (int v = lane; v < V; v += 64) { const float e = expf(lg[v] * inv_temp - mx); sp[v] = e; sum += e; }
  sum = wave_sum(sum);
  for (int v = lane; v < V; v += 64) sp[v] = sp[v] / sum;
  __builtin_amdgcn_fence(__ATOMIC_RELEASE, "wavefront");
  __builtin_amdgcn_wave_barrier();
  for (int v = lane; v < V; v += 64) {
    const float p = sp[v];
    int rank = 0;
    for (int u = 0; u < V; ++u) { const float q = sp[u]; rank += (q > p || (q == p && u < v)) ? 1 : 0; }
    ss[rank] = p; si[rank] = v;
  }
  __builtin_amdgcn_fence(__ATOMIC_RELEASE, "wavefront");
  __builtin_amdgcn_wave_barrier();
  int tok = 0;
  if (lane == 0) {
    int K = V;
    if (top_p > 0.f && top_p < 1.f) {
      float cum = 0.f;
      K = 1;
      for (int k = 0; k + 1 < V; ++k) {
        cum += ss[k];
        if (cum > top_p) break;
        K = k + 2;
      }
    }
    float S = 0.f;
    for (int k = 0; k < K; ++k) S += ss[k];
    const unsigned long long r = mix64(mix64(seed ^ mix64(key)) + (unsigned long long)ctr);
    const float u = (float)(r >> 40) * (1.0f / 16777216.0f);
    const float target = u * S;
    float acc = 0.f;
    tok = si[K - 1];
    for (int k = 0; k < K; ++k) { acc += ss[k]; if (target < acc) { tok = si[k]; break; } }
  }
  return __shfl(tok, 0, 64);
}

#ifdef ETD_HEAD_STAMP
__device__ long long g_head_stamp[8 * 16];
#define HSTAMP(i) do { if (tid == 0 && blockIdx.x < 8) g_head_stamp[blockIdx.x * 16 + (i)] = clock64(); } while (0)
#else
#define HSTAMP(i) do { } while (0)
#endif
#define DH_LDX 520
#define DH_LDL 257
__global__ __launch_bounds__(512) void k_dstep_head(const float* p_hfin, int p_M, const int* p_row_slot, const int* p_row_active, const int* p_row_pos, DHeadArgs a) {
  __shared__ __attribute__((aligned(16))) d16 Xs[32 * DH_LDX];
  __shared__ float Ls[32 * DH_LDL];
  __shared__ float sps[8][256], sss[8][256];
  __shared__ int sis[8][256];
  const int tid = threadIdx.x, lane = tid & 63, wave = __builtin_amdgcn_readfirstlane(tid >> 6), r = lane & 31, h = lane >> 5;
  const int m0 = blockIdx.x * 32, H = a.H;
  const float inv_temp = a.samp ? a.samp->inv_temp : 0.f;
  HSTAMP(0);
  const int k8 = lane * 8;
  f32x4 hv0[4], hv1[4];
#pragma unroll
  for (int j = 0; j < 4; ++j) {
    int gm = m0 + wave * 4 + j; gm = gm < p_M ? gm : p_M - 1;
    const float* xp = p_hfin + (long long)gm * H;
    hv0[j] = *reinterpret_cast<const f32x4*>(xp + lane * 4); hv1[j] = *reinterpret_cast<const f32x4*>(xp + lane * 4 + 256);
  }
  int mapv;
  {
    const int j = lane & 3, f = lane >> 2;
    int gm = m0 + wave * 4 + j; gm = gm < p_M ? gm : p_M - 1;
    const int* mp = f == 0 ? p_row_slot : (f == 1 ? p_row_active : p_row_pos);
    mapv = mp[gm];
  }
  f32x4 lg_[2], lb_[2];
#pragma unroll
  for (int half = 0; half < 2; ++half) {
    lg_[half] = *reinterpret_cast<const f32x4*>(a.lnf_g + lane * 4 + half * 256); lb_[half] = *reinterpret_cast<const f32x4*>(a.lnf_b + lane * 4 + half * 256);
  }
  __builtin_amdgcn_sched_barrier(0);
  d16x8 wf[32];
  {
    const bool own = wave * 32 < a.Vpad;
    const d16* wfr = a.Whead + (own ? ((long long)wave * 32 * 64 + lane) * 8 : 0);
#pragma unroll
    for (int s4 = 0; s4 < 32; ++s4) wf[s4] = *reinterpret_cast<const d16x8*>(wfr + s4 * 64 * 8);
  }
  __builtin_amdgcn_sched_barrier(0);
  {
    float s4[4], q4[4], mean[4];
#pragma unroll
    for (int j = 0; j < 4; ++j) {
      const f32x4 v0 = hv0[j], v1 = hv1[j];
      float s = 0.f;
      s += v0[0] + v0[1] + v0[2] + v0[3];
      s += v1[0] + v1[1] + v1[2] + v1[3];
      s4[j] = s;
    }
    wave_sum_n<4>(s4);
    HSTAMP(6);
// ... 763 lines not shown
      const drsrc_t ys = d_rsrc(g.Y, (long long)g.k_splits * p_M * 512 * 4);
      const int vo = ((bz * p_M + m) * 512 + n0 + 4 * h) * 4;
#pragma unroll
      for (int q = 0; q < 4; ++q) {
        const f32x4 o4 = {acc[4 * q], acc[4 * q + 1], acc[4 * q + 2], acc[4 * q + 3]};
        __builtin_amdgcn_raw_buffer_store_b128(__builtin_bit_cast(u32x4, o4), ys, vo + 32 * q, 0, D_SC1);
      }
    }
    asm volatile("s_waitcnt vmcnt(0)" ::: "memory");
    SS(2); SS_FLUSH(2, 1);
    int old = -1;
    if (h == 0 && m < p_M) old = D_ARRIVE(fin.cnt + m);
    unsigned long long last = __ballot(old == fin.target - 1);
    while (last) {
      const int rl = __builtin_ctzll(last);
      last &= last - 1;
      row_finish(fin, m0 + rl, p_M, lane);
      if (lane == 0) D_CNT_RESET(fin.cnt + m0 + rl);
    }
  } else {
    if (m >= p_M) return;
    DGemmArgs b = g;
    b.Y = g.Y + (long long)bz * p_M * g.ldy;
    dgemm_epilogue<true, DEPI_PARTIAL>(b, acc, m, n0, h);
    SS(2); SS_FLUSH(2, 1);
  }
}

template <int NW, bool FIN, bool PAIR = false>
__global__ __launch_bounds__(64 * NW) __attribute__((amdgpu_waves_per_eu(FIN ? ETD_FIN_OCC : (PAIR ? ETD_AD_OCC : AdOcc<NW>::lo), AdOcc<NW>::hi))) void k_dstep_attn_down(const int* p_row_sp, const float* p_Q, const void* p_Kc, const void* p_Vc, long long p_slot_stride,
                                                         int p_max_ctx, int p_n_heads, float p_scale, int p_identity, int p_gemm_wgs, int p_M,
                                                         DAttnArgs a, DGemmArgs g, DRowFin fin) {
  attn_stamp_begin(a.stamp, a.stamp_par, (int)blockIdx.x);
  dstep_attn_down_body<NW, FIN, PAIR>(p_row_sp, p_Q, p_Kc, p_Vc, p_slot_stride, p_max_ctx, p_n_heads, p_scale, p_identity, p_gemm_wgs, p_M, a, g, fin);
  attn_stamp_end(a.stamp, a.stamp_par, (int)blockIdx.x);
}

static int ad_waves(int M) {
  (void)M;
#ifdef ETD_EXPERIMENTS
  static const int env = getenv("ETD_AD_WAVES") ? atoi(getenv("ETD_AD_WAVES")) : 0;
  return (env == 8 || env == 16) ? env : 4;
#else
  return 4;
#endif
}
int launch_dstep_attn_down(const DAttnArgs& a, const DGemmArgs& g, const DRowFin* fin, hipStream_t st) {
#ifndef ETD_EXPERIMENTS
  if (fin) ETD_FAIL(ETD_EINVAL, "dstep_attn_down: the in-launch row finish is built with -DETD_EXPERIMENTS only");
#endif
  if (fin && (!fin->cnt || fin->target != a.n_heads + 16 * g.k_splits || fin->nslab != 12 || g.k_splits + a.n_heads != 12 || fin->P != g.Y ||
              a.dense_out != g.Y + (size_t)g.k_splits * a.M * 512 || !fin->bias || !fin->hin || !fin->hout || fin->hin == fin->hout || (fin->x1 && (!fin->x2 || !fin->g1 || !fin->b1 || !fin->g2 || !fin->b2))))
    ETD_FAIL(ETD_EINVAL, "dstep_attn_down: bad row-finish arguments");
  if (a.M < 1 || a.M > DS_STEP_MAX_ROWS || a.n_heads < 1 || !a.row_sp || !a.dense_w || !a.dense_out || a.max_ctx < 256 ||
      g.M != a.M || !g.Xb || !g.W || !g.Y || g.ldy != 512 || g.N != 512 || g.Npad != 512 || g.k_splits < 1 || g.k_splits * 512 > g.K || (g.K % 8) || a.n_heads * 64 != 512)
    ETD_FAIL(ETD_EINVAL, "dstep_attn_down: bad arguments");
  static const int pair_env = ETD_XENV("ETD_AD_PAIR") ? atoi(ETD_XENV("ETD_AD_PAIR")) : -1;
  const bool pair = (pair_env < 0 ? a.pair != 0 : pair_env > 0) && !fin && ad_waves(a.M) == 4;
  const int nw = pair ? 8 : ad_waves(a.M), units = nw / 2;
  const int RT = (a.M + 31) / 32, FT = g.Npad / 32;
  const int slots = ((FT * g.k_splits + 7) / 8) * RT;
  const int gemm_wgs = ((slots + units - 1) / units) * 8;
  ProfScope ps("k_dstep_attn_down", st, 2.0 * a.M * 512 * (512.0 * g.k_splits + 512.0), a.bytes_hint + 512.0 * (512.0 * g.k_splits + 512.0) * 2);
  const DRowFin f0 = fin ? *fin : DRowFin{};
#define ETD_AD_LAUNCH(NW_, FIN_) hipLaunchKernelGGL((k_dstep_attn_down<NW_, FIN_>), dim3(gemm_wgs + a.M * a.n_heads), dim3(64 * NW_), 0, st, a.row_sp, a.Q, a.Kc, a.Vc, a.slot_stride, a.max_ctx, a.n_heads, a.scale, \
                                              a.identity ? 1 : 0, gemm_wgs, a.M, a, g, f0)
  if (pair) {
    hipLaunchKernelGGL((k_dstep_attn_down<8, false, true>), dim3(gemm_wgs + ((a.M + 1) / 2) * a.n_heads), dim3(512), 0, st, a.row_sp, a.Q, a.Kc, a.Vc, a.slot_stride, a.max_ctx, a.n_heads, a.scale,
                       a.identity ? 1 : 0, gemm_wgs, a.M, a, g, f0);
  } else
#ifdef ETD_EXPERIMENTS
  if (fin) { if (nw == 16) ETD_AD_LAUNCH(16, true); else if (nw == 8) ETD_AD_LAUNCH(8, true); else ETD_AD_LAUNCH(4, true); }
  else if (nw == 16) ETD_AD_LAUNCH(16, false); else if (nw == 8) ETD_AD_LAUNCH(8, false); else ETD_AD_LAUNCH(4, false);
#else
  ETD_AD_LAUNCH(4, false);
#endif
#undef ETD_AD_LAUNCH
  HIP_TRY(hipGetLastError());
  return ETD_OK;
}

int launch_dattn(const DAttnArgs& a, bool kv_bf16, hipStream_t st) {
  if (a.M <= 0) ETD_FAIL(ETD_EINVAL, "dattn: bad M");
  ProfScope ps(a.M > 512 ? "k_dattn_prefill" : "k_dattn", st, 0, a.bytes_hint);
  dim3 g(a.M, a.n_heads);
  const int ident = a.identity && a.row_sp && a.max_ctx >= 64 ? 1 : 0;
  if (kv_bf16) hipLaunchKernelGGL(k_dattn<d16>, g, dim3(256), 0, st, a.row_sp, a.Q, a.Kc, a.Vc, a.slot_stride, a.max_ctx, a.n_heads, a.scale, ident, a);
  else hipLaunchKernelGGL(k_dattn<float>, g, dim3(256), 0, st, a.row_sp, a.Q, a.Kc, a.Vc, a.slot_stride, a.max_ctx, a.n_heads, a.scale, ident, a);
  HIP_TRY(hipGetLastError());
  return ETD_OK;
}

__global__ __launch_bounds__(256) void k_ln_rows(const float* __restrict__ hsrc, int M, int H, const float* __restrict__ g1, const float* __restrict__ b1,
                                                 const float* __restrict__ g2, const float* __restrict__ b2, float eps, d16* __restrict__ x1, d16* __restrict__ x2) {
  const int lane = threadIdx.x & 63, row = blockIdx.x * 4 + (threadIdx.x >> 6);
  if (row >= M) return;
  const float* xp = hsrc + (long long)row * H;
  float v[4][8];
  float s = 0.f;
#pragma unroll
  for (int it = 0; it < 4; ++it) {
    const int k = lane * 8 + it * 512;
    if (k < H) {
      const f32x4 a = *reinterpret_cast<const f32x4*>(xp + k), b = *reinterpret_cast<const f32x4*>(xp + k + 4);
      v[it][0] = a[0]; v[it][1] = a[1]; v[it][2] = a[2]; v[it][3] = a[3]; v[it][4] = b[0]; v[it][5] = b[1]; v[it][6] = b[2]; v[it][7] = b[3];
#pragma unroll
      for (int j = 0; j < 8; ++j) s += v[it][j];
    }
  }
  s = wave_sum(s);
  const float mean = s / (float)H;
  float q = 0.f;
#pragma unroll
  for (int it = 0; it < 4; ++it)
    if (lane * 8 + it * 512 < H) {
#pragma unroll
      for (int j = 0; j < 8; ++j) { const float d0 = v[it][j] - mean; q += d0 * d0; }
    }
  q = wave_sum(q);
  const float rstd = rsqrtf(q / (float)H + eps);
#pragma unroll
  for (int it = 0; it < 4; ++it) {
    const int k = lane * 8 + it * 512;
    if (k < H) {
      const f32x4 ga = *reinterpret_cast<const f32x4*>(g1 + k), gb = *reinterpret_cast<const f32x4*>(g1 + k + 4);
      const f32x4 ba = *reinterpret_cast<const f32x4*>(b1 + k), bb = *reinterpret_cast<const f32x4*>(b1 + k + 4);
      d16x8 o1;
#pragma unroll
      for (int j = 0; j < 4; ++j) { o1[j] = (d16)((v[it][j] - mean) * rstd * ga[j] + ba[j]); o1[4 + j] = (d16)((v[it][4 + j] - mean) * rstd * gb[j] + bb[j]); }
      *reinterpret_cast<d16x8*>(x1 + (long long)row * H + k) = o1;
      if (x2) {
        const f32x4 ha = *reinterpret_cast<const f32x4*>(g2 + k), hb = *reinterpret_cast<const f32x4*>(g2 + k + 4);
        const f32x4 ca = *reinterpret_cast<const f32x4*>(b2 + k), cb = *reinterpret_cast<const f32x4*>(b2 + k + 4);
        d16x8 o2;
#pragma unroll
        for (int j = 0; j < 4; ++j) { o2[j] = (d16)((v[it][j] - mean) * rstd * ha[j] + ca[j]); o2[4 + j] = (d16)((v[it][4 + j] - mean) * rstd * hb[j] + cb[j]); }
        *reinterpret_cast<d16x8*>(x2 + (long long)row * H + k) = o2;
      }
    }
  }
}
int launch_ln_rows(const float* hsrc, int M, int H, const float* g1, const float* b1, const float* g2, const float* b2, float eps,
                   d16* x1, d16* x2, hipStream_t st) {
  if (M <= 0 || H % 8 || H > 2048) ETD_FAIL(ETD_EINVAL, "ln_rows: bad shape");
  ProfScope ps("k_ln_rows", st, 0, (double)M * H * (4 + (x2 ? 4 : 2)));
  hipLaunchKernelGGL(k_ln_rows, dim3((M + 3) / 4), dim3(256), 0, st, hsrc, M, H, g1, b1, g2, b2, eps, x1, x2);
  HIP_TRY(hipGetLastError());
  return ETD_OK;
}

#ifndef ETD_RL_ROWS
#define ETD_RL_ROWS 4
#endif
template <int KS>
__global__ __launch_bounds__(64 * ETD_RL_ROWS) void k_resid_ln_rows(const float* __restrict__ P, int ks_rt, const float* __restrict__ bias, const float* __restrict__ add,
                                                       const float* __restrict__ hin, float* __restrict__ hout, int M, int H,
                                                       const float* __restrict__ g1, const float* __restrict__ b1, const float* __restrict__ g2,
                                                       const float* __restrict__ b2, float eps, d16* __restrict__ x1, d16* __restrict__ x2) {
  const int lane = threadIdx.x & 63, row = blockIdx.x * ETD_RL_ROWS + (threadIdx.x >> 6);
  if (row >= M) return;
  SS_DECL(); SS(0);
  const long long ro = (long long)row * H;
  float v[4][8];
  float s = 0.f;
  const int k0 = lane * 8;
  f32x4 pg1[2], pb1[2], pg2[2], pb2[2];
  if (x1 && k0 < H) {
#pragma unroll
    for (int hh = 0; hh < 2; ++hh) {
      pg1[hh] = *reinterpret_cast<const f32x4*>(g1 + k0 + 4 * hh); pb1[hh] = *reinterpret_cast<const f32x4*>(b1 + k0 + 4 * hh);
      pg2[hh] = *reinterpret_cast<const f32x4*>(g2 + k0 + 4 * hh); pb2[hh] = *reinterpret_cast<const f32x4*>(b2 + k0 + 4 * hh);
    }
  }
#pragma unroll
  for (int it = 0; it < 4; ++it) {
    const int k = lane * 8 + it * 512;
    if (k < H) {
      float acc[8];
#pragma unroll
      for (int j = 0; j < 8; ++j) acc[j] = 0.f;
      if constexpr (KS > 0) {
        f32x4 pa[KS], pb[KS];
#pragma unroll
        for (int z = 0; z < KS; ++z) {
          const float* pp = P + (long long)z * M * H + ro + k;
          pa[z] = *reinterpret_cast<const f32x4*>(pp); pb[z] = *reinterpret_cast<const f32x4*>(pp + 4);
        }
#pragma unroll
        for (int z = 0; z < KS; ++z)
#pragma unroll
          for (int j = 0; j < 4; ++j) { acc[j] += pa[z][j]; acc[4 + j] += pb[z][j]; }
      } else {
        for (int z = 0; z < ks_rt; ++z) {
          const float* pp = P + (long long)z * M * H + ro + k;
          const f32x4 a = *reinterpret_cast<const f32x4*>(pp), b = *reinterpret_cast<const f32x4*>(pp + 4);
#pragma unroll
          for (int j = 0; j < 4; ++j) { acc[j] += a[j]; acc[4 + j] += b[j]; }
        }
      }
      const f32x4 ba = *reinterpret_cast<const f32x4*>(bias + k), bb = *reinterpret_cast<const f32x4*>(bias + k + 4);
      f32x4 da = {0.f, 0.f, 0.f, 0.f}, db = {0.f, 0.f, 0.f, 0.f};
      if (add) { da = *reinterpret_cast<const f32x4*>(add + ro + k); db = *reinterpret_cast<const f32x4*>(add + ro + k + 4); }
      const f32x4 ha = *reinterpret_cast<const f32x4*>(hin + ro + k), hb = *reinterpret_cast<const f32x4*>(hin + ro + k + 4);
#pragma unroll
      for (int j = 0; j < 4; ++j) { v[it][j] = ((acc[j] + ba[j]) + da[j]) + ha[j]; v[it][4 + j] = ((acc[4 + j] + bb[j]) + db[j]) + hb[j]; }
      const f32x4 oa = {v[it][0], v[it][1], v[it][2], v[it][3]}, ob = {v[it][4], v[it][5], v[it][6], v[it][7]};
      *reinterpret_cast<f32x4*>(hout + ro + k) = oa;
      *reinterpret_cast<f32x4*>(hout + ro + k + 4) = ob;
#pragma unroll
      for (int j = 0; j < 8; ++j) s += v[it][j];
    }
  }
  if (!x1) return;
  SS(1);
  s = wave_sum(s);
  const float mean = s / (float)H;
  float q = 0.f;
#pragma unroll
  for (int it = 0; it < 4; ++it)
    if (lane * 8 + it * 512 < H) {
#pragma unroll
      for (int j = 0; j < 8; ++j) { const float d0 = v[it][j] - mean; q += d0 * d0; }
    }
  q = wave_sum(q);
  const float rstd = rsqrtf(q / (float)H + eps);
  SS(2);
#pragma unroll
  for (int it = 0; it < 4; ++it) {
    const int k = lane * 8 + it * 512;
    if (k < H) {
      d16x8 o1, o2;
#pragma unroll
      for (int j = 0; j < 8; ++j) {
        const float n = (v[it][j] - mean) * rstd;
        const float w1 = it == 0 ? pg1[j >> 2][j & 3] : g1[k + j], c1 = it == 0 ? pb1[j >> 2][j & 3] : b1[k + j];
        const float w2 = it == 0 ? pg2[j >> 2][j & 3] : g2[k + j], c2 = it == 0 ? pb2[j >> 2][j & 3] : b2[k + j];
        o1[j] = (d16)(n * w1 + c1);
        o2[j] = (d16)(n * w2 + c2);
      }
      *reinterpret_cast<d16x8*>(x1 + ro + k) = o1;
      *reinterpret_cast<d16x8*>(x2 + ro + k) = o2;
    }
  }
  SS(3); SS_FLUSH(3, 0);
}
int launch_resid_ln_rows(const float* P, int k_splits, const float* bias, const float* add, const float* hin, float* hout, int M, int H,
                         const float* g1, const float* b1, const float* g2, const float* b2, float eps, d16* x1, d16* x2, hipStream_t st) {
  if (M <= 0 || H % 8 || H > 2048 || k_splits < 1) ETD_FAIL(ETD_EINVAL, "resid_ln_rows: bad shape");
  ProfScope ps("k_resid_ln_rows", st, 0, (double)M * H * 4 * (k_splits + 3));
  if (k_splits == 5) hipLaunchKernelGGL(k_resid_ln_rows<5>, dim3((M + ETD_RL_ROWS - 1) / ETD_RL_ROWS), dim3(64 * ETD_RL_ROWS), 0, st, P, k_splits, bias, add, hin, hout, M, H, g1, b1, g2, b2, eps, x1, x2);
  else if (k_splits == 12) hipLaunchKernelGGL(k_resid_ln_rows<12>, dim3((M + ETD_RL_ROWS - 1) / ETD_RL_ROWS), dim3(64 * ETD_RL_ROWS), 0, st, P, k_splits, bias, add, hin, hout, M, H, g1, b1, g2, b2, eps, x1, x2);
  else hipLaunchKernelGGL(k_resid_ln_rows<0>, dim3((M + ETD_RL_ROWS - 1) / ETD_RL_ROWS), dim3(64 * ETD_RL_ROWS), 0, st, P, k_splits, bias, add, hin, hout, M, H, g1, b1, g2, b2, eps, x1, x2);
  HIP_TRY(hipGetLastError());
  return ETD_OK;
}

__global__ void k_gather_rows(const float* __restrict__ src, const int* __restrict__ idx, int n, int H, float* __restrict__ out) {
  const int i = blockIdx.x;
  const float* sp = src + (long long)idx[i] * H;
  for (int k = threadIdx.x * 4; k < H; k += blockDim.x * 4) *reinterpret_cast<f32x4*>(out + (long long)i * H + k) = *reinterpret_cast<const f32x4*>(sp + k);
}
int launch_gather_rows(const float* src, const int* idx, int n, int H, float* out, hipStream_t st) {
  hipLaunchKernelGGL(k_gather_rows, dim3(n), dim3(128), 0, st, src, idx, n, H, out);
  HIP_TRY(hipGetLastError());
  return ETD_OK;
}

__global__ void k_dembed(DEmbedArgs a) {
  const int m = blockIdx.x;
  int id, cl, at[4];
  if (a.ids) {
    id = a.ids[m]; cl = a.cls[m];
#pragma unroll
    for (int k = 0; k < 4; ++k) at[k] = a.attrs[k * a.M + m];
  } else {
    const int slot = a.slots ? a.slots[m] : a.rows.slot[m];
    if (a.slots && threadIdx.x == 0) {
      const int ps = a.len[slot];
      a.row_slot_out[m] = slot; a.row_pos_out[m] = ps; a.row_active_out[m] = a.done[slot] ? 0 : 1;
      if (a.row_sp_out) { a.row_sp_out[2 * m] = slot; a.row_sp_out[2 * m + 1] = ps; }
    }
    id = a.cur_tok[slot]; cl = a.tgt_cls;
#pragma unroll
    for (int k = 0; k < 4; ++k) at[k] = a.tgt_attrs[slot * 4 + k];
  }
  for (int i = threadIdx.x; i < a.H; i += blockDim.x) {
    float p = a.attr_tab[(0 * a.n_bins + at[0]) * a.H + i];
    p += a.attr_tab[(1 * a.n_bins + at[1]) * a.H + i];
    p += a.attr_tab[(2 * a.n_bins + at[2]) * a.H + i];
    p += a.attr_tab[(3 * a.n_bins + at[3]) * a.H + i];
    a.h[(long long)m * a.H + i] = (a.word[(long long)id * a.H + i] + a.cls_emb[cl * a.H + i]) + p;
  }
}
int launch_dembed(const DEmbedArgs& a, hipStream_t st) {
  hipLaunchKernelGGL(k_dembed, dim3(a.M), dim3(256), 0, st, a);
  HIP_TRY(hipGetLastError());
  return ETD_OK;
}

__global__ void k_dargmax(DArgmaxArgs a) {
  __shared__ float sp[256], ss[256];
  __shared__ int si[256];
  const int m = blockIdx.x, lane = threadIdx.x;
  const float* lg = a.logits + (long long)m * a.ldl;
  const int slot_r = a.rows.slot[m];
  const float inv_temp = a.samp ? a.samp->inv_temp : 0.f;
  int bi;
  if (inv_temp > 0.f) bi = wave_sample(lg, a.V, lane, inv_temp, a.samp->top_p, a.samp->seed, a.rng_key[slot_r], (unsigned)a.n_out[slot_r], sp, ss, si);
  else bi = wave_argmax(lg, a.V, lane);
  if (lane == 0 && a.rows.active[m]) {
    const int slot = slot_r;
    if (!a.done[slot]) {
      const int n = a.n_out[slot];
      if (n < a.out_cap) a.out_tok[(long long)slot * a.out_cap + n] = bi;
      a.n_out[slot] = n + 1;
      a.cur_tok[slot] = bi;
      a.len[slot] = a.rows.pos[m] + 1;
      if (bi == a.eos[slot] || n + 1 >= a.limit[slot]) a.done[slot] = 1;
    }
  }
}
int launch_dargmax(const DArgmaxArgs& a, hipStream_t st) {
  if (a.samp && (a.V > 256 || !a.rng_key)) ETD_FAIL(ETD_EINVAL, "dargmax: sampling needs a vocabulary <= 256 and stream keys");
  hipLaunchKernelGGL(k_dargmax, dim3(a.M), dim3(64), 0, st, a);
  HIP_TRY(hipGetLastError());
  return ETD_OK;
}
```

### etude_amd/csrc/dec_prefill.hip

```cpp
#include "dec_kernels.h"
#include "prof.h"

#include <cstdlib>

#define PA_LDK 72
#define PA_LDV 96

typedef __attribute__((ext_vector_type(4))) short pa_s16x4;
typedef __attribute__((address_space(3))) pa_s16x4* pa_lds_s16x4;

__global__ __launch_bounds__(256) void k_pattn(PAttnArgs a) {
  __shared__ __attribute__((aligned(16))) unsigned char smem[64 * PA_LDK * 2 + 64 * PA_LDV * 2];
  d16* Ks = reinterpret_cast<d16*>(smem);
  d16* Vs = Ks + 64 * PA_LDK;
  const int tid = threadIdx.x, lane = tid & 63, wave = __builtin_amdgcn_readfirstlane(tid >> 6), r = lane & 31, h = lane >> 5;
  const int nh = a.n_heads;
  const int seq = blockIdx.y / nh, head = blockIdx.y - seq * nh;
  const int S = a.seq_len[seq];
  const long long r0 = a.seq_row0[seq];
  const int off = (128 - (S & 127)) & 127;
  if ((int)blockIdx.x * 128 - off >= S) return;
  const int slot = a.row_slot[r0];
  const int q0 = (int)blockIdx.x * 128 + wave * 32 - off;
  int qi = q0 + r; const bool qvalid = qi >= 0 && qi < S; qi = qi < 0 ? 0 : (qi < S ? qi : S - 1);

  const d16* qp = a.Q + (r0 + qi) * a.ldq + head * 64;
  d16x8 qf[4];
#pragma unroll
  for (int s = 0; s < 4; ++s) qf[s] = *reinterpret_cast<const d16x8*>(qp + s * 16 + h * 8);

  const long long cbase = (long long)slot * a.slot_stride + (long long)head * a.max_ctx * 64;
  const d16* kbase = a.Kc + cbase;
  const d16* vbase = a.Vc + cbase;

  f32x16 o[2];
#pragma unroll
  for (int t = 0; t < 2; ++t)
#pragma unroll
    for (int i = 0; i < 16; ++i) o[t][i] = 0.f;
  float mrun = -INFINITY, lrun = 0.f;

  int ntile = (S + 63) >> 6;
  { const int lim = ((int)blockIdx.x * 128 + 127 - off) / 64 + 1; ntile = ntile < lim ? ntile : lim; }
  u32x4 kreg[2], vreg[2];
  auto tile_gload = [&](int kv0_) {
#pragma unroll
    for (int i = 0; i < 2; ++i) {
      const int c = tid + i * 256, row = c >> 3, ch = c & 7;
      int key = kv0_ + row; key = key < S ? key : S - 1;
      kreg[i] = *reinterpret_cast<const u32x4*>(kbase + (long long)key * 64 + ch * 8);
      vreg[i] = *reinterpret_cast<const u32x4*>(vbase + (long long)key * 64 + ch * 8);
    }
  };
  const int tq = (lane >> 2) & 3, tp = lane & 3, tg = (lane >> 4) & 1;
  const d16* vtr = Vs + (4 * h + tq) * PA_LDV + 16 * tg + 4 * tp;
  tile_gload(0);
  for (int jt = 0; jt < ntile; ++jt) {
    const int kv0 = jt * 64;
#pragma unroll
    for (int i = 0; i < 2; ++i) {
      const int c = tid + i * 256, row = c >> 3, ch = c & 7;
      *reinterpret_cast<u32x4*>(Ks + row * PA_LDK + ch * 8) = kreg[i];
      *reinterpret_cast<u32x4*>(Vs + row * PA_LDV + ch * 8) = vreg[i];
    }
    __syncthreads();
    if (jt + 1 < ntile) tile_gload(kv0 + 64);
    if (kv0 <= q0 + 31) {
      f32x16 sT[2];
#pragma unroll
      for (int kt = 0; kt < 2; ++kt) {
#pragma unroll
        for (int i = 0; i < 16; ++i) sT[kt][i] = 0.f;
#pragma unroll
        for (int s = 0; s < 4; ++s) {
          const d16x8 kf = *reinterpret_cast<const d16x8*>(Ks + (kt * 32 + r) * PA_LDK + s * 16 + h * 8);
          sT[kt] = mfma32(kf, qf[s], sT[kt]);
        }
      }
      const bool need_mask = (kv0 + 64 > S) || (kv0 + 63 > q0);
      float mx = -INFINITY;
      if (need_mask) {
#pragma unroll
        for (int kt = 0; kt < 2; ++kt)
#pragma unroll
          for (int i = 0; i < 16; ++i) {
            const int key = kv0 + kt * 32 + acc_row(i, h);
            const float v = (key < S && key <= qi) ? sT[kt][i] : -INFINITY;
            sT[kt][i] = v;
            mx = fmaxf(mx, v);
          }
      } else {
#pragma unroll
        for (int kt = 0; kt < 2; ++kt)
#pragma unroll
          for (int i = 0; i < 16; ++i) mx = fmaxf(mx, sT[kt][i]);
      }
      mx = fmaxf(mx, xhalf(mx));
      const float mnew = fmaxf(mrun, mx);
      const float c = a.scale_log2e;
      const float alpha = __builtin_amdgcn_exp2f((mrun - mnew) * c);
      mrun = mnew;
      const float mc = -mnew * c;
      float ps = 0.f;
#pragma unroll
      for (int kt = 0; kt < 2; ++kt)
#pragma unroll
        for (int i = 0; i < 16; ++i) { const float p = __builtin_amdgcn_exp2f(fmaf(sT[kt][i], c, mc)); sT[kt][i] = p; ps += p; }
      lrun = lrun * alpha + ps;
#pragma unroll
      for (int t = 0; t < 2; ++t)
#pragma unroll
        for (int i = 0; i < 16; ++i) o[t][i] *= alpha;
#pragma unroll
      for (int ks = 0; ks < 4; ++ks) {
        d16x8 pf;
#pragma unroll
        for (int j = 0; j < 8; ++j) pf[j] = (d16)sT[ks >> 1][8 * (ks & 1) + j];
#pragma unroll
        for (int dt = 0; dt < 2; ++dt) {
          const pa_s16x4 lo = __builtin_amdgcn_ds_read_tr16_b64_v4i16((pa_lds_s16x4)(vtr + (ks * 16) * PA_LDV + dt * 32));
          const pa_s16x4 hi = __builtin_amdgcn_ds_read_tr16_b64_v4i16((pa_lds_s16x4)(vtr + (ks * 16 + 8) * PA_LDV + dt * 32));
          const __attribute__((ext_vector_type(8))) short v8 = {lo[0], lo[1], lo[2], lo[3], hi[0], hi[1], hi[2], hi[3]};
          o[dt] = mfma32(__builtin_bit_cast(d16x8, v8), pf, o[dt]);
        }
      }
    }
    __syncthreads();
  }

  lrun += xhalf(lrun);
  const float inv = 1.f / lrun;
  if (qvalid) {
    d16* op = a.O + (r0 + q0 + r) * a.ldo + head * 64;
#pragma unroll
    for (int dt = 0; dt < 2; ++dt)
#pragma unroll
      for (int q = 0; q < 4; ++q) {
        const int d = dt * 32 + 8 * q + 4 * h;
        *reinterpret_cast<d16x4*>(op + d) = pack4d(o[dt][4 * q] * inv, o[dt][4 * q + 1] * inv, o[dt][4 * q + 2] * inv, o[dt][4 * q + 3] * inv);
      }
  }
}

int launch_pattn(const PAttnArgs& a, hipStream_t st) {
  if (a.n_seq <= 0 || a.max_len <= 0 || a.n_heads <= 0 || !a.Q || !a.Kc || !a.Vc || !a.O || !a.seq_row0 || !a.seq_len || !a.row_slot || a.max_len > a.max_ctx ||
      (a.ldq % 8) || (a.ldo % 4) || (((uintptr_t)a.Q | (uintptr_t)a.Kc | (uintptr_t)a.Vc) & 15) || ((uintptr_t)a.O & 7))
    ETD_FAIL(ETD_EINVAL, "pattn: bad arguments");
  ETD_LAUNCH_FILTER("k_pattn");
  ProfScope ps("k_pattn", st, a.flops_hint, ((double)a.n_seq * 4.0 * a.max_len * 64 * a.n_heads) * 2);
  dim3 g((a.max_len + 127) / 128, a.n_seq * a.n_heads);
  hipLaunchKernelGGL(k_pattn, g, dim3(256), 0, st, a);
  HIP_TRY(hipGetLastError());
  return ETD_OK;
}

#define PQ_EPP 136
#define PQ_TILE_ELEMS (32 * 512)
typedef const __attribute__((address_space(1))) void* pq_gptr_t;
typedef __attribute__((address_space(3))) void* pq_lptr_t;

template <int NW>
__global__ __launch_bounds__(64 * NW) void k_pqkv(PQkvArgs a) {
  __shared__ __attribute__((aligned(16))) unsigned char smem[2 * PQ_TILE_ELEMS * 2 + NW * 32 * PQ_EPP * 2 + 1536 * 4];
  d16* ring = reinterpret_cast<d16*>(smem);
  d16* stg_all = reinterpret_cast<d16*>(smem + 2 * PQ_TILE_ELEMS * 2);
  float* sb = reinterpret_cast<float*>(smem + 2 * PQ_TILE_ELEMS * 2 + NW * 32 * PQ_EPP * 2);
  const int tid = threadIdx.x, lane = tid & 63, wave = __builtin_amdgcn_readfirstlane(tid >> 6), r = lane & 31, h = lane >> 5;
  d16* stg = stg_all + wave * (32 * PQ_EPP);
  const int NT = a.N >> 5;
  const int mw = blockIdx.x * (32 * NW) + wave * 32;
  const int m = mw + r, mc = m < a.M ? m : a.M - 1;

  auto issue = [&](int t) {
    constexpr int PW = 32 / NW;
    const d16* src = a.Wf + (long long)t * PQ_TILE_ELEMS + wave * (PW * 512) + lane * 8;
    d16* dst = ring + (t & 1) * PQ_TILE_ELEMS + wave * (PW * 512);
    __builtin_amdgcn_global_load_lds((pq_gptr_t)src, (pq_lptr_t)dst, 16, 0, 0);
    __builtin_amdgcn_global_load_lds((pq_gptr_t)src, (pq_lptr_t)dst, 16, 1024, 0);
    __builtin_amdgcn_global_load_lds((pq_gptr_t)src, (pq_lptr_t)dst, 16, 2048, 0);
    __builtin_amdgcn_global_load_lds((pq_gptr_t)src, (pq_lptr_t)dst, 16, 3072, 0);
    if constexpr (PW == 8) {
      __builtin_amdgcn_global_load_lds((pq_gptr_t)(src + 2048), (pq_lptr_t)(dst + 2048), 16, 0, 0);
      __builtin_amdgcn_global_load_lds((pq_gptr_t)(src + 2048), (pq_lptr_t)(dst + 2048), 16, 1024, 0);
      __builtin_amdgcn_global_load_lds((pq_gptr_t)(src + 2048), (pq_lptr_t)(dst + 2048), 16, 2048, 0);
      __builtin_amdgcn_global_load_lds((pq_gptr_t)(src + 2048), (pq_lptr_t)(dst + 2048), 16, 3072, 0);
    }
  };
  issue(0);
  for (int i = tid; i < a.N; i += 64 * NW) sb[i] = a.bias[i];
  d16x8 xf[32];
  {
    const d16* xp = a.X + (long long)mc * a.ldx + 8 * h;
#pragma unroll
    for (int s = 0; s < 32; ++s) xf[s] = *reinterpret_cast<const d16x8*>(xp + 16 * s);
  }
  const int pos_l = a.rows.pos[mc];
  const f32x4 c4 = *reinterpret_cast<const f32x4*>(a.rope_cos + (long long)pos_l * 8 + 4 * h);
  const f32x4 s4 = *reinterpret_cast<const f32x4*>(a.rope_sin + (long long)pos_l * 8 + 4 * h);
  const int er8 = lane >> 3, ec8 = lane & 7;
  long long qoff[4], coff[4];
#pragma unroll
  for (int it = 0; it < 4; ++it) {
    const int mr = mw + it * 8 + er8, mrc = mr < a.M ? mr : a.M - 1;
    const int rpos = a.rows.pos[mrc], rslot = a.rows.slot[mrc], ract = a.rows.active[mrc];
    qoff[it] = mr < a.M ? (long long)mr * (a.n_heads * 64) + ec8 * 8 : -1;
    coff[it] = (mr < a.M && ract && rpos < a.max_ctx) ? (long long)rslot * a.slot_stride + (long long)rpos * 64 + ec8 * 8 : -1;
  }
  const unsigned ring_l = (unsigned)reinterpret_cast<uintptr_t>(ring) + lane * 16;

  auto store_block = [&](int u) {
    const int head = u / 3, part = u - head * 3;
    d16* cbase = (part == 1 ? a.Kc : a.Vc) + (long long)head * a.max_ctx * 64;
#pragma unroll
    for (int it = 0; it < 4; ++it) {
      const u32x4 val = *reinterpret_cast<const u32x4*>(stg + (it * 8 + er8) * PQ_EPP + ec8 * 8);
      if (part == 0) { if (qoff[it] >= 0) *reinterpret_cast<u32x4*>(a.Qb + qoff[it] + head * 64) = val; }
      else if (coff[it] >= 0) *reinterpret_cast<u32x4*>(cbase + coff[it]) = val;
    }
  };
#define PQ_RD4(buf, F0)                                                                                                  \
  do {                                                                                                                   \
    asm volatile("ds_read_b128 %0, %1 offset:%2" : "=v"(buf[0]) : "v"(sl), "n"((F0) * 1024));                            \
    asm volatile("ds_read_b128 %0, %1 offset:%2" : "=v"(buf[1]) : "v"(sl), "n"((F0) * 1024 + 1024));                     \
    asm volatile("ds_read_b128 %0, %1 offset:%2" : "=v"(buf[2]) : "v"(sl), "n"((F0) * 1024 + 2048));                     \
    asm volatile("ds_read_b128 %0, %1 offset:%2" : "=v"(buf[3]) : "v"(sl), "n"((F0) * 1024 + 3072));                     \
  } while (0)
#define PQ_MFMA(c, af, bfr) asm volatile(ETD_MFMA16_DEC " %0, %1, %2, %0" : "+v"(c) : "v"(af), "v"(bfr))
#define PQ_MFMA0(c, af, bfr) asm volatile(ETD_MFMA16_DEC " %0, %1, %2, 0" : "=&v"(c) : "v"(af), "v"(bfr))
#define PQ_GROUP(c, G)                                                                                                   \
  do {                                                                                                                   \
    if constexpr ((G) < 7) { PQ_RD4(wf[((G) + 1) & 1], ((G) + 1) * 4); asm volatile("s_waitcnt lgkmcnt(4)" ::: "memory"); } \
    else asm volatile("s_waitcnt lgkmcnt(0)" ::: "memory");                                                              \
    if constexpr ((G) == 0) PQ_MFMA0(c, wf[0][0], xf[0]); else PQ_MFMA(c, wf[(G) & 1][0], xf[4 * (G)]);                  \
    PQ_MFMA(c, wf[(G) & 1][1], xf[4 * (G) + 1]);                                                                         \
    PQ_MFMA(c, wf[(G) & 1][2], xf[4 * (G) + 2]);                                                                         \
    PQ_MFMA(c, wf[(G) & 1][3], xf[4 * (G) + 3]);                                                                         \
    __builtin_amdgcn_sched_barrier(0);                                                                                   \
  } while (0)
#define PQ_TILE(c, t)                                                                                                    \
  do {                                                                                                                   \
    asm volatile("s_waitcnt vmcnt(0) lgkmcnt(0)" ::: "memory");    \
    __syncthreads();                                               \
    if ((t) + 1 < NT) issue((t) + 1);                                                                                    \
    if ((t) >= 2 && !((t) & 1)) store_block(((t) - 2) >> 1);                                                              \
    const unsigned sl = ring_l + ((t) & 1) * (PQ_TILE_ELEMS * 2);                                                        \
    d16x8 wf[2][4];                                                                                                     \
    asm volatile("s_waitcnt lgkmcnt(0)" ::: "memory");             \
    __builtin_amdgcn_sched_barrier(0);                                                                                   \
    PQ_RD4(wf[0], 0);                                                                                                    \
    PQ_GROUP(c, 0); PQ_GROUP(c, 1); PQ_GROUP(c, 2); PQ_GROUP(c, 3); PQ_GROUP(c, 4); PQ_GROUP(c, 5); PQ_GROUP(c, 6); PQ_GROUP(c, 7); \
  } while (0)
  for (int u = 0; u < (NT >> 1); ++u) {
    f32x16 c0, c1;
    PQ_TILE(c0, 2 * u);
    PQ_TILE(c1, 2 * u + 1);
    asm volatile("s_nop 15\n\ts_nop 15" : "+v"(c1) : : "memory");
    {
      const int part = u % 3;
      float v[2][16];
#pragma unroll
      for (int i = 0; i < 16; ++i) { v[0][i] = c0[i] + sb[64 * u + acc_row(i, h)]; v[1][i] = c1[i] + sb[64 * u + 32 + acc_row(i, h)]; }
      if (part < 2) {
#pragma unroll
        for (int i = 0; i < 4; ++i) {
          const float x1 = v[0][i], x2 = v[0][i + 4];
          v[0][i] = x1 * c4[i] - x2 * s4[i];
          v[0][i + 4] = x2 * c4[i] + x1 * s4[i];
        }
      }
#pragma unroll
      for (int nn = 0; nn < 2; ++nn)
#pragma unroll
        for (int q = 0; q < 4; ++q)
          *reinterpret_cast<d16x4*>(stg + r * PQ_EPP + nn * 32 + 8 * q + 4 * h) = pack4d(v[nn][4 * q], v[nn][4 * q + 1], v[nn][4 * q + 2], v[nn][4 * q + 3]);
    }
  }
#undef PQ_TILE
#undef PQ_GROUP
#undef PQ_MFMA
#undef PQ_MFMA0
#undef PQ_RD4
  store_block((NT >> 1) - 1);
}

int launch_pqkv(const PQkvArgs& a, hipStream_t st) {
  if (a.M <= 0 || a.N != 1536 || a.ldx < 512 || (a.ldx % 8) || !a.X || !a.Wf || !a.bias || !a.Qb || !a.Kc || !a.Vc || !a.rows.pos || !a.rows.slot || !a.rows.active ||
      !a.rope_cos || !a.rope_sin || a.n_heads != 8 || (((uintptr_t)a.X | (uintptr_t)a.Wf | (uintptr_t)a.Qb | (uintptr_t)a.Kc | (uintptr_t)a.Vc) & 15) || (a.slot_stride % 8))
    ETD_FAIL(ETD_EINVAL, "pqkv: bad arguments");
  ETD_LAUNCH_FILTER("k_pqkv");
  ProfScope ps("k_pqkv", st, 2.0 * a.M * a.N * 512.0, ((double)a.M * 512 + (double)a.N * 512 + 3.0 * a.M * 512) * 2);
  static const int nw = getenv("ETD_PQKV_WAVES") ? atoi(getenv("ETD_PQKV_WAVES")) : 8;
  if (nw == 4) hipLaunchKernelGGL(k_pqkv<4>, dim3((a.M + 127) / 128), dim3(256), 0, st, a);
  else hipLaunchKernelGGL(k_pqkv<8>, dim3((a.M + 255) / 256), dim3(512), 0, st, a);
  HIP_TRY(hipGetLastError());
  return ETD_OK;
}
```

### include/etude_hip_debug.h

```cpp
#ifndef ETUDE_HIP_DEBUG_H
#define ETUDE_HIP_DEBUG_H
#include "etude_hip.h"

#ifdef __cplusplus
extern "C" {
#endif

int etd_debug_boundary_cost(int n_nodes, int iters, int big_args, void* stream, double* eager_us, double* graph_us);
int etd_debug_linear(int M, int N, int K, int iters, void* stream, double* us);
int etd_debug_kernel_loop(int which, int iters, void* stream);
int etd_debug_empty_launch(int gx, int gy, int gz, int* sink_dev, void* stream);

int etd_extractor_debug_vel_logits(etd_ext*, float* vel_logits_dev);
int etd_extractor_debug_tap(etd_ext*, int stage, void* dst_dev);

int etd_debug_assemble_prompt(const etd_sched_cfg* cfg, int n_hist, const int32_t* const* hx, const int32_t* hxn, const int32_t* const* hy,
                              const int32_t* hyn, const int32_t* hattrs4, const int32_t* x, int xn, const int32_t* y_attrs4,
                              int32_t* ids_out, int32_t* cls_out, int32_t* attrs4_out, int cap, int* T_out);
int etd_debug_assemble_scored(const etd_sched_cfg* cfg, int n_hist, const int32_t* const* hx, const int32_t* hxn, const int32_t* const* hy,
                              const int32_t* hyn, const int32_t* hattrs4, const int32_t* x, int xn, const int32_t* y, int yn, const int32_t* y_attrs4,
                              int32_t* ids_out, int32_t* cls_out, int32_t* attrs4_out, int32_t* labels_out, int cap, int* T_out);

int etd_debug_decoder_checksum(etd_dec*, unsigned long long* out, int cap, void* stream);
int etd_debug_decoder_kv_rowsums(etd_dec*, unsigned* out_host, long long cap, void* stream);
int etd_debug_decoder_trace_begin(etd_dec*, int cap_steps, void* stream);
int etd_debug_decoder_trace_slabs(etd_dec*, float* out_host, long long cap_floats, int n_active, void* stream);
int etd_debug_decoder_trace_lanes(etd_dec*, float* out_host, long long cap_floats, int n_active, void* stream);
int etd_debug_decoder_trace_q(etd_dec*, float* out_host, long long cap_floats, int n_active, void* stream);
int etd_debug_decoder_peek_kv(etd_dec*, int layer, int slot, int head, int n_pos, unsigned short* k_out, unsigned short* v_out, void* stream);
int etd_debug_decoder_trace_read(etd_dec*, unsigned* out_host, long long cap_words, int n_active, int* steps_done, void* stream);

int etd_debug_decoder_force_pair(etd_dec*, int mode);
int etd_debug_decoder_step_logits(etd_dec*, int on, float* out_host, int n_active, void* stream);

int etd_debug_gemm3(const float* x_dev, int M, int K, const float* w_host, const float* bias_host, int N, float x_bound, int gelu, float* y_dev,
                    const float* ln_g_host, const float* ln_b_host, void* stream);
enum { ETD_G3_KERNEL_AUTO = 0 , ETD_G3_KERNEL_TILE = 1 , ETD_G3_KERNEL_SMALL = 2  };
enum { ETD_G3_EPI_BIAS = 0, ETD_G3_EPI_GELU = 1, ETD_G3_EPI_RESID = 2, ETD_G3_EPI_LOGITS = 3, ETD_G3_EPI_QKV = 4, ETD_G3_EPI_RELU = 6 };
typedef struct etd_debug_g3_case {
  int struct_bytes;
  int kernel, epi;
  int M, N, K, ldx, ldy;
  const float* X; long long x_elems;
  const float* W; const float* bias;
  float x_bound;
  const float* ln_g; const float* ln_b; float ln_eps;
  float* Y; long long y_elems;
  const float* add; const float* hin; float* hout; long long h_elems;
  const int32_t* pos; const int32_t* slot; const int32_t* active;
  int n_heads, max_ctx, n_slots, rope_rows;
  const float* rope_cos; const float* rope_sin;
  float* Q; long long q_elems;
  float* Kc; float* Vc; long long kv_elems;
} etd_debug_g3_case;
int etd_debug_gemm3_case(const etd_debug_g3_case* c, void* stream);
int etd_debug_ln_rows_f32(const float* h_dev, int M, int H, const float* g1_host, const float* b1_host, const float* g2_host, const float* b2_host, float eps,
                          float* x1_dev, float* x2_dev, void* stream);
int etd_debug_g3_pack(const float* W, int N, int K, uint16_t* planes_out, long long cap, long long* n_out, int32_t* log2_out);

int etd_debug_attn3(const float* q_dev, const float* k_dev, const float* v_dev, float* o_dev, int n_seq, int n_heads, int Sq, int Sk, float q_bound, float k_bound, float v_bound,
                    int causal, const int32_t* lens_host, void* stream);

int etd_debug_g3_bounds(const float* W, const float* c, int N, int K, const float* g, const float* b, float elem_bound, float* out4, int32_t* log2_out4);

int etd_beat_debug_taps(etd_beat*, float* front_dev, float* layer0_dev);

int etd_dbn_debug_viterbi(etd_dbn*, int hmm_index, const double* densities_dev, long long T, int32_t* path_out, double* logprob_out);

#ifdef __cplusplus
}
#endif
#endif
```

Before: 588.4.

## Add K/V-only prefill QKV for last layer, 64-row QKV-up kernel, configurable LN rows

In the last prefill layer only the last rows' queries are needed, so the prefill QKV kernel gets a kv_only mode that skips the Q weight tiles and writes only K/V into the cache, removing a third of that GEMM. A new 64-row-tile, 512-thread decode-step QKV+up kernel is used for mid-size batches (216–512 rows), aiming at better CU utilisation than the 128-row tile. The residual-LN kernel gains a templated rows-per-workgroup parameter, selectable by environment variable, and debug peek entry points are added. The new paths add code complexity and carry some risk in the tile remapping.

```diff
diff --git a/etude_amd/_lib.py b/etude_amd/_lib.py
--- a/etude_amd/_lib.py
+++ b/etude_amd/_lib.py
@@ -200,6 +200,9 @@
     "etd_dbn_track": (C.c_int, [C.c_void_p, C.c_void_p, C.c_int, C.c_int, c_i64_p, C.c_void_p, C.c_longlong, C.c_void_p, C.c_void_p, C.c_void_p, C.c_longlong,
                                 C.c_void_p, C.c_void_p, C.POINTER(C.c_longlong), C.c_void_p]),
     "etd_dbn_debug_viterbi": (C.c_int, [C.c_void_p, C.c_int, C.c_void_p, C.c_longlong, C.c_void_p, C.POINTER(C.c_double)]),
+    "etd_debug_decoder_peek": (C.c_int, [C.c_void_p, C.c_int, C.c_int, C.c_int, C.c_int, C.c_void_p, C.c_longlong, C.c_void_p]),
+    "etd_debug_resid_ln_rows": (C.c_int, [C.c_void_p, C.c_int, C.c_void_p, C.c_void_p, C.c_void_p, C.c_void_p, C.c_int, C.c_int, C.c_void_p, C.c_void_p, C.c_void_p, C.c_void_p,
+                                          C.c_float, C.c_void_p, C.c_void_p, C.c_void_p]),
     "etd_debug_decoder_trace_read": (C.c_int, [C.c_void_p, C.c_void_p, C.c_longlong, C.c_int, C.POINTER(C.c_int), C.c_void_p]),
 }
 
diff --git a/etude_amd/csrc/api_dec.hip b/etude_amd/csrc/api_dec.hip
--- a/etude_amd/csrc/api_dec.hip
+++ b/etude_amd/csrc/api_dec.hip
@@ -353,7 +353,7 @@
   return ETD_OK;
 }
 
-static int prefill16_qkv(etd_dec* d, int l, const float* hin, const DecRows& rows, int M, bool mfma_attn, hipStream_t st) {
+static int prefill16_qkv(etd_dec* d, int l, const float* hin, const DecRows& rows, int M, bool mfma_attn, bool kv_only, hipStream_t st) {
   const Layer& w = d->layers[l];
   DGemmArgs q = qkv_args(d, l, hin, rows, M); q.Xb = d->X1b; q.Y = d->qkv_raw; q.ldy = 3 * d->H;
   if (mfma_attn) q.Qb = d->Qb;
@@ -361,6 +361,7 @@
   if (!(mfma_attn && pqkv_on && M >= 49152 && d->H == 512 && d->nh == 8 && w.qkv.N == 1536)) return linear16(w.qkv, d->X1b, M, q, DEPI_QKV, st);
   PQkvArgs pa = {};
   pa.X = d->X1b; pa.ldx = d->H; pa.Wf = (const d16*)w.qkv.Wf; pa.bias = w.qkv.b; pa.M = M; pa.N = w.qkv.N; pa.rows = rows;
+  pa.kv_only = kv_only && !getenv("ETD_NO_PQKV_KVONLY");
   pa.rope_cos = d->rope_cos; pa.rope_sin = d->rope_sin; pa.Qb = d->Qb; pa.Kc = (d16*)q.Kc; pa.Vc = (d16*)q.Vc; pa.slot_stride = d->slot_stride; pa.max_ctx = d->ctx; pa.n_heads = d->nh;
   return launch_pqkv(pa, st);
 }
@@ -400,7 +401,7 @@
   float* hin = d->h; float* hout = d->h2;
   for (int l = 0; l < d->L; ++l) {
     if (l == 0 || !fmlp) ETD_TRY(ln_rows16(d, l, hin, M, st));
-    ETD_TRY(prefill16_qkv(d, l, hin, rows, M, pf != nullptr, st));
+    ETD_TRY(prefill16_qkv(d, l, hin, rows, M, pf != nullptr, tail && l == d->L - 1, st));
     ETD_TRY(tail && l == d->L - 1 ? prefill16_last_rows(d, *lo, hin, hout, st) : prefill16_layer_rest(d, l, rows, M, pf, fmlp, hin, hout, st));
     std::swap(hin, hout);
   }
@@ -1365,6 +1366,29 @@
   HIP_TRY(hipStreamSynchronize(st));
   return ETD_OK;
 }
+extern "C" int etd_debug_decoder_peek(etd_dec* d, int what, int layer, int pos0, int n_pos, void* out_host, long long cap_bytes, void* stream) {
+  hipStream_t st = (hipStream_t)stream;
+  if (!d || !d->bf16w || !out_host || what < 0 || what > 3) ETD_FAIL(ETD_EINVAL, "decoder_peek: bad args");
+  if (what == 0) {
+    if (cap_bytes < (long long)d->S * d->H * 4) ETD_FAIL(ETD_ENOMEM, "decoder_peek: buffer too small");
+    HIP_TRY(hipMemcpyAsync(out_host, d->Q, (size_t)d->S * d->H * 4, hipMemcpyDeviceToHost, st));
+  } else if (what == 1) {
+    if (!d->Xcat || cap_bytes < (long long)d->S * d->I * 2) ETD_FAIL(ETD_ENOMEM, "decoder_peek: buffer too small");
+    HIP_TRY(hipMemcpy2DAsync(out_host, (size_t)d->I * 2, d->Xcat, (size_t)(d->I + d->H) * 2, (size_t)d->I * 2, d->S, hipMemcpyDeviceToHost, st));
+  } else {
+    if (layer < 0 || layer >= d->L || pos0 < 0 || n_pos < 1 || pos0 + n_pos > d->ctx || d->slot_stride != (long long)d->nh * d->ctx * 64) ETD_FAIL(ETD_EINVAL, "decoder_peek: bad cache range");
+    if (cap_bytes < (long long)d->S * d->nh * n_pos * 128) ETD_FAIL(ETD_ENOMEM, "decoder_peek: buffer too small");
+    const char* src = (const char*)kv_layer(d, what == 2 ? d->Kc : d->Vc, layer) + (size_t)pos0 * 128;
+    HIP_TRY(hipMemcpy2DAsync(out_host, (size_t)n_pos * 128, src, (size_t)d->ctx * 128, (size_t)n_pos * 128, (size_t)d->S * d->nh, hipMemcpyDeviceToHost, st));
+  }
+  HIP_TRY(hipStreamSynchronize(st));
+  return ETD_OK;
+}
+extern "C" int etd_debug_resid_ln_rows(const float* P, int k_splits, const float* bias, const float* add, const float* hin, float* hout, int M, int H, const float* g1,
+                                       const float* b1, const float* g2, const float* b2, float eps, void* x1, void* x2, void* stream) {
+  if (!P || !bias || !hin || !hout || (x1 && !(g1 && b1 && g2 && b2 && x2))) ETD_FAIL(ETD_EINVAL, "debug_resid_ln_rows: bad args");
+  return launch_resid_ln_rows(P, k_splits, bias, add, hin, hout, M, H, g1, b1, g2, b2, eps, (d16*)x1, (d16*)x2, (hipStream_t)stream);
+}
 extern "C" int etd_debug_decoder_trace_read(etd_dec* d, unsigned* out_host, long long cap_words, int n_active, int* steps_done, void* stream) {
   hipStream_t st = (hipStream_t)stream;
   if (!d || !d->trace || !out_host || !steps_done || n_active < 1 || n_active > d->S) ETD_FAIL(ETD_EINVAL, "trace_read: bad args");
diff --git a/etude_amd/csrc/dec_kernels.h b/etude_amd/csrc/dec_kernels.h
--- a/etude_amd/csrc/dec_kernels.h
+++ b/etude_amd/csrc/dec_kernels.h
@@ -124,6 +124,7 @@
   const float* rope_cos; const float* rope_sin;
   d16* Qb;
   d16* Kc; d16* Vc; long long slot_stride; int max_ctx, n_heads;
+  int kv_only;
 };
 int launch_pqkv(const PQkvArgs& a, hipStream_t st);
 
diff --git a/etude_amd/csrc/dec_kernels.hip b/etude_amd/csrc/dec_kernels.hip
--- a/etude_amd/csrc/dec_kernels.hip
+++ b/etude_amd/csrc/dec_kernels.hip
@@ -552,6 +552,144 @@
   }
 }
 
+__global__ __launch_bounds__(512) __attribute__((amdgpu_waves_per_eu(2, 4))) void k_dstep_qkv_up_m64(int p_M, int split128, int p_ftiles128, const d16* p_Wfq, const d16* p_Wfu, const d16* p_Xq, const d16* p_Xu,
+                                                          int p_ldxq, int p_ldxu, DGemmArgs q, DGemmArgs up) {
+  __shared__ __attribute__((aligned(16))) unsigned char smem[4 * 64 * QMT_PITCH];
+  const int tid = threadIdx.x, lane = tid & 63, wave = tid >> 6, r = lane & 31, h = lane >> 5, kh = wave >> 2, w4 = wave & 3, fh = w4 & 1, rh = w4 >> 1, gt = tid & 255;
+  const int M = p_M, K = 512;
+  const int RT = (M + 63) / 64, bid = blockIdx.x, ft = ((bid >> 3) / RT) * 8 + (bid & 7);
+  if (ft >= p_ftiles128) return;
+  const bool isq = ft < split128;
+  const int mwg = ((bid >> 3) % RT) * 64, m0 = mwg + rh * 32, n0 = (isq ? ft : ft - split128) * 128 + fh * 64;
+  const d16* wfrag = (isq ? p_Wfq : p_Wfu) + ((long long)(n0 / 32) * (K / 16) * 64 + lane) * 8;
+  const d16* xbase = (isq ? p_Xq : p_Xu) + kh * 256;
+  const int ldx = isq ? p_ldxq : p_ldxu;
+  int xsrc[2], xdst[2];
+#pragma unroll
+  for (int i = 0; i < 2; ++i) {
+    const int pce = gt + 256 * i, row = pce >> 3, c = pce & 7;
+    int gmr = mwg + row; gmr = gmr < M ? gmr : M - 1;
+    xsrc[i] = gmr * ldx + c * 8;
+    xdst[i] = row * QMT_PITCH + c * 16;
+  }
+  int gm = m0 + r; gm = gm < M ? gm : M - 1;
+  const int pos = q.rows.pos[gm], slot = q.rows.slot[gm], act = q.rows.active[gm];
+  f32x4 bq[2][4];
+#pragma unroll
+  for (int f = 0; f < 2; ++f) {
+    const float* bp = (isq ? q.bias : up.bias) + n0 + 32 * f + 4 * h;
+#pragma unroll
+    for (int q4 = 0; q4 < 4; ++q4) bq[f][q4] = *reinterpret_cast<const f32x4*>(bp + 8 * q4);
+  }
+  f32x16 acc[2];
+#pragma unroll
+  for (int f = 0; f < 2; ++f)
+#pragma unroll
+    for (int i = 0; i < 16; ++i) acc[f][i] = 0.f;
+  u32x4 xr[2];
+  d16x8 wf[2][4][2];
+  auto xrequest = [&](int cc) {
+#pragma unroll
+    for (int i = 0; i < 2; ++i) xr[i] = *reinterpret_cast<const u32x4*>(xbase + xsrc[i] + cc * 64);
+  };
+  auto wrequest = [&](int cc, int b) {
+#pragma unroll
+    for (int s4 = 0; s4 < 4; ++s4)
+#pragma unroll
+      for (int f = 0; f < 2; ++f) wf[b][s4][f] = *reinterpret_cast<const d16x8*>(wfrag + (long long)((f * 32 + (kh * 4 + cc) * 4 + s4) * 64) * 8);
+  };
+  unsigned char* xh = smem + kh * (2 * 64 * QMT_PITCH);
+  xrequest(0); wrequest(0, 0);
+#pragma unroll
+  for (int cc = 0; cc < 4; ++cc) {
+    const int b = cc & 1;
+    unsigned char* xb = xh + b * (64 * QMT_PITCH);
+#pragma unroll
+    for (int i = 0; i < 2; ++i) *reinterpret_cast<u32x4*>(xb + xdst[i]) = xr[i];
+    __syncthreads();
+    if (cc + 1 < 4) { xrequest(cc + 1); wrequest(cc + 1, b ^ 1); }
+#pragma unroll
+    for (int s4 = 0; s4 < 4; ++s4) {
+      const d16x8 xf = *reinterpret_cast<const d16x8*>(xb + (rh * 32 + r) * QMT_PITCH + s4 * 32 + h * 16);
+#pragma unroll
+      for (int f = 0; f < 2; ++f) acc[f] = mfma32(wf[b][s4][f], xf, acc[f]);
+    }
+  }
+  __syncthreads();
+  float* xch = reinterpret_cast<float*>(smem + w4 * 8192);
+  if (kh == 1) {
+#pragma unroll
+    for (int f = 0; f < 2; ++f)
+#pragma unroll
+      for (int q4 = 0; q4 < 4; ++q4) {
+        const f32x4 o = {acc[f][4 * q4], acc[f][4 * q4 + 1], acc[f][4 * q4 + 2], acc[f][4 * q4 + 3]};
+        *reinterpret_cast<f32x4*>(xch + ((f * 4 + q4) * 64 + lane) * 4) = o;
+      }
+  }
+  __syncthreads();
+  if (kh == 1) return;
+  unsigned char* sw = smem + w4 * 8192;
+  const int head = n0 / 192, part = (n0 - head * 192) >> 6;
+  const int er = lane >> 3, ec = lane & 7;
+  float vv[2][16];
+#pragma unroll
+  for (int f = 0; f < 2; ++f) {
+    const bool rope = isq && part < 2 && f == 0;
+    f32x16 a2;
+#pragma unroll
+    for (int q4 = 0; q4 < 4; ++q4) {
+      const f32x4 o = *reinterpret_cast<const f32x4*>(xch + ((f * 4 + q4) * 64 + lane) * 4);
+#pragma unroll
+      for (int j = 0; j < 4; ++j) a2[4 * q4 + j] = acc[f][4 * q4 + j] + o[j];
+    }
+    f32x4 rc = {1.f, 1.f, 1.f, 1.f}, rs = {0.f, 0.f, 0.f, 0.f};
+    if (rope) {
+      rc = *reinterpret_cast<const f32x4*>(q.rope_cos + (long long)pos * 8 + 4 * h);
+      rs = *reinterpret_cast<const f32x4*>(q.rope_sin + (long long)pos * 8 + 4 * h);
+    }
+    qkv_up_tile_values(a2, bq[f], isq, rope, rc, rs, vv[f]);
+  }
+  __builtin_amdgcn_wave_barrier();
+  if (!isq || part != 0) {
+#pragma unroll
+    for (int f = 0; f < 2; ++f)
+#pragma unroll
+      for (int q4 = 0; q4 < 4; ++q4)
+        *reinterpret_cast<d16x4*>(sw + r * QMT_PITCH + (32 * f + 8 * q4 + 4 * h) * 2) = pack4d(vv[f][4 * q4], vv[f][4 * q4 + 1], vv[f][4 * q4 + 2], vv[f][4 * q4 + 3]);
+    __builtin_amdgcn_wave_barrier();
+#pragma unroll
+    for (int it = 0; it < 4; ++it) {
+      const int row = it * 8 + er, m = m0 + row;
+      const u32x4 val = *reinterpret_cast<const u32x4*>(sw + row * QMT_PITCH + ec * 16);
+      const int ps = __shfl(pos, row, 64), sl = __shfl(slot, row, 64), ac = __shfl(act, row, 64);
+      if (m >= M) continue;
+      if (!isq) {
+        if (n0 + ec * 8 < up.N) *reinterpret_cast<u32x4*>(up.Yb + (long long)m * up.ldy + n0 + ec * 8) = val;
+      } else {
+        if (ac && ps < q.max_ctx)
+          *reinterpret_cast<u32x4*>(reinterpret_cast<d16*>(part == 1 ? q.Kc : q.Vc) + (long long)sl * q.slot_stride + ((long long)head * q.max_ctx + ps) * 64 + ec * 8) = val;
+      }
+    }
+  } else {
+#pragma unroll
+    for (int f = 0; f < 2; ++f) {
+#pragma unroll
+      for (int q4 = 0; q4 < 4; ++q4) {
+        const f32x4 o = {vv[f][4 * q4], vv[f][4 * q4 + 1], vv[f][4 * q4 + 2], vv[f][4 * q4 + 3]};
+        *reinterpret_cast<f32x4*>(sw + r * QMT_PITCH + (8 * q4 + 4 * h) * 4) = o;
+      }
+      __builtin_amdgcn_wave_barrier();
+#pragma unroll
+      for (int it = 0; it < 4; ++it) {
+        const int row = it * 8 + er, m = m0 + row;
+        const u32x4 val = *reinterpret_cast<const u32x4*>(sw + row * QMT_PITCH + ec * 16);
+        if (m < M) *reinterpret_cast<u32x4*>(q.Q + (long long)m * (q.n_heads * 64) + head * 64 + 32 * f + ec * 4) = val;
+      }
+      __builtin_amdgcn_wave_barrier();
+    }
+  }
+}
+
 int launch_dstep_qkv_up(const DGemmArgs& q, const DGemmArgs& up, hipStream_t st) {
   if (q.M != up.M || q.K != up.K || q.M < 1 || q.M > DS_STEP_MAX_ROWS || !q.Xb || !up.Xb || !up.Yb || q.K != 512 || q.Npad % 32 || up.Npad % 32 ||
       q.rot_half != 8 || q.N % 192 || q.Qb || !q.Q || !q.bias || !up.bias || up.N % 4)
@@ -561,9 +699,19 @@
   const int ftiles = split + up.Npad / 32;
   static const bool mt_on = !(ETD_XENV("ETD_QKV_MT") && atoi(ETD_XENV("ETD_QKV_MT")) == 0);
   static const int mt_min = ETD_XENV("ETD_QKV_MT_MIN") ? atoi(ETD_XENV("ETD_QKV_MT_MIN")) : 256;
-  if (mt_on && q.M >= mt_min && q.Npad % 128 == 0 && up.Npad % 128 == 0 && q.Wf && up.Wf) {
-    const int split128 = q.Npad / 128, ft128 = split128 + up.Npad / 128, RT128 = (q.M + 127) / 128;
-    hipLaunchKernelGGL(k_dstep_qkv_up_mt, dim3((unsigned)(((ft128 + 7) / 8) * 8 * RT128)), dim3(256), 0, st, q.M, split128, ft128, (const d16*)q.Wf, (const d16*)up.Wf, q.Xb, up.Xb, q.ldx, up.ldx, q, up);
+  constexpr int QKV_M64_MIN_ROWS = 216, QKV_M64_MAX_ROWS = 512;
+  const int form = getenv("ETD_QKV_FORM") ? atoi(getenv("ETD_QKV_FORM")) : 0;
+  const bool mt_fits = q.Npad % 128 == 0 && up.Npad % 128 == 0 && q.Wf && up.Wf;
+  const bool m64 = form ? form == 64 : q.M >= QKV_M64_MIN_ROWS && q.M <= QKV_M64_MAX_ROWS;
+  if (form != 32 && mt_fits && (form ? true : mt_on && (m64 || q.M >= mt_min))) {
+    const int split128 = q.Npad / 128, ft128 = split128 + up.Npad / 128;
+    if (m64) {
+      const int RT64 = (q.M + 63) / 64;
+      hipLaunchKernelGGL(k_dstep_qkv_up_m64, dim3((unsigned)(((ft128 + 7) / 8) * 8 * RT64)), dim3(512), 0, st, q.M, split128, ft128, (const d16*)q.Wf, (const d16*)up.Wf, q.Xb, up.Xb, q.ldx, up.ldx, q, up);
+    } else {
+      const int RT128 = (q.M + 127) / 128;
+      hipLaunchKernelGGL(k_dstep_qkv_up_mt, dim3((unsigned)(((ft128 + 7) / 8) * 8 * RT128)), dim3(256), 0, st, q.M, split128, ft128, (const d16*)q.Wf, (const d16*)up.Wf, q.Xb, up.Xb, q.ldx, up.ldx, q, up);
+    }
     HIP_TRY(hipGetLastError());
     return ETD_OK;
   }
@@ -1633,12 +1781,12 @@
 #ifndef ETD_RL_ROWS
 #define ETD_RL_ROWS 4
 #endif
-template <int KS>
-__global__ __launch_bounds__(64 * ETD_RL_ROWS) void k_resid_ln_rows(const float* __restrict__ P, int ks_rt, const float* __restrict__ bias, const float* __restrict__ add,
+template <int KS, int ROWS>
+__global__ __launch_bounds__(64 * ROWS) void k_resid_ln_rows(const float* __restrict__ P, int ks_rt, const float* __restrict__ bias, const float* __restrict__ add,
                                                        const float* __restrict__ hin, float* __restrict__ hout, int M, int H,
                                                        const float* __restrict__ g1, const float* __restrict__ b1, const float* __restrict__ g2,
                                                        const float* __restrict__ b2, float eps, d16* __restrict__ x1, d16* __restrict__ x2) {
-  const int lane = threadIdx.x & 63, row = blockIdx.x * ETD_RL_ROWS + (threadIdx.x >> 6);
+  const int lane = threadIdx.x & 63, row = blockIdx.x * ROWS + (threadIdx.x >> 6);
   if (row >= M) return;
   SS_DECL(); SS(0);
   const long long ro = (long long)row * H;
@@ -1725,13 +1873,30 @@
   }
   SS(3); SS_FLUSH(3, 0);
 }
+static inline int rl_rows_for(int ) {
+  if (const char* e = getenv("ETD_RL_ROWS_PER_WG")) { const int v = atoi(e); if (v == 1 || v == 2 || v == ETD_RL_ROWS) return v; }
+  return ETD_RL_ROWS;
+}
+template <int KS, int ROWS>
+static void resid_ln_rows_launch(const float* P, int k_splits, const float* bias, const float* add, const float* hin, float* hout, int M, int H,
+                                 const float* g1, const float* b1, const float* g2, const float* b2, float eps, d16* x1, d16* x2, hipStream_t st) {
+  hipLaunchKernelGGL((k_resid_ln_rows<KS, ROWS>), dim3((M + ROWS - 1) / ROWS), dim3(64 * ROWS), 0, st, P, k_splits, bias, add, hin, hout, M, H, g1, b1, g2, b2, eps, x1, x2);
+}
+template <int KS>
+static void resid_ln_rows_pick(int rows, const float* P, int k_splits, const float* bias, const float* add, const float* hin, float* hout, int M, int H,
+                               const float* g1, const float* b1, const float* g2, const float* b2, float eps, d16* x1, d16* x2, hipStream_t st) {
+  if (rows == 1) resid_ln_rows_launch<KS, 1>(P, k_splits, bias, add, hin, hout, M, H, g1, b1, g2, b2, eps, x1, x2, st);
+  else if (rows == 2) resid_ln_rows_launch<KS, 2>(P, k_splits, bias, add, hin, hout, M, H, g1, b1, g2, b2, eps, x1, x2, st);
+  else resid_ln_rows_launch<KS, ETD_RL_ROWS>(P, k_splits, bias, add, hin, hout, M, H, g1, b1, g2, b2, eps, x1, x2, st);
+}
 int launch_resid_ln_rows(const float* P, int k_splits, const float* bias, const float* add, const float* hin, float* hout, int M, int H,
                          const float* g1, const float* b1, const float* g2, const float* b2, float eps, d16* x1, d16* x2, hipStream_t st) {
   if (M <= 0 || H % 8 || H > 2048 || k_splits < 1) ETD_FAIL(ETD_EINVAL, "resid_ln_rows: bad shape");
   ProfScope ps("k_resid_ln_rows", st, 0, (double)M * H * 4 * (k_splits + 3));
-  if (k_splits == 5) hipLaunchKernelGGL(k_resid_ln_rows<5>, dim3((M + ETD_RL_ROWS - 1) / ETD_RL_ROWS), dim3(64 * ETD_RL_ROWS), 0, st, P, k_splits, bias, add, hin, hout, M, H, g1, b1, g2, b2, eps, x1, x2);
-  else if (k_splits == 12) hipLaunchKernelGGL(k_resid_ln_rows<12>, dim3((M + ETD_RL_ROWS - 1) / ETD_RL_ROWS), dim3(64 * ETD_RL_ROWS), 0, st, P, k_splits, bias, add, hin, hout, M, H, g1, b1, g2, b2, eps, x1, x2);
-  else hipLaunchKernelGGL(k_resid_ln_rows<0>, dim3((M + ETD_RL_ROWS - 1) / ETD_RL_ROWS), dim3(64 * ETD_RL_ROWS), 0, st, P, k_splits, bias, add, hin, hout, M, H, g1, b1, g2, b2, eps, x1, x2);
+  const int rows = rl_rows_for(M);
+  if (k_splits == 5) resid_ln_rows_pick<5>(rows, P, k_splits, bias, add, hin, hout, M, H, g1, b1, g2, b2, eps, x1, x2, st);
+  else if (k_splits == 12) resid_ln_rows_pick<12>(rows, P, k_splits, bias, add, hin, hout, M, H, g1, b1, g2, b2, eps, x1, x2, st);
+  else resid_ln_rows_pick<0>(rows, P, k_splits, bias, add, hin, hout, M, H, g1, b1, g2, b2, eps, x1, x2, st);
   HIP_TRY(hipGetLastError());
   return ETD_OK;
 }
diff --git a/etude_amd/csrc/dec_prefill.hip b/etude_amd/csrc/dec_prefill.hip
--- a/etude_amd/csrc/dec_prefill.hip
+++ b/etude_amd/csrc/dec_prefill.hip
@@ -159,7 +159,9 @@
 typedef const __attribute__((address_space(1))) void* pq_gptr_t;
 typedef __attribute__((address_space(3))) void* pq_lptr_t;
 
-template <int NW>
+template <bool KV> __device__ __forceinline__ int pq_block(int j) { return KV ? 3 * (j >> 1) + 1 + (j & 1) : j; }
+template <bool KV> __device__ __forceinline__ int pq_tile(int n) { return 2 * pq_block<KV>(n >> 1) + (n & 1); }
+template <int NW, bool KV>
 __global__ __launch_bounds__(64 * NW) void k_pqkv(PQkvArgs a) {
   __shared__ __attribute__((aligned(16))) unsigned char smem[2 * PQ_TILE_ELEMS * 2 + NW * 32 * PQ_EPP * 2 + 1536 * 4];
   d16* ring = reinterpret_cast<d16*>(smem);
@@ -167,13 +169,13 @@
   float* sb = reinterpret_cast<float*>(smem + 2 * PQ_TILE_ELEMS * 2 + NW * 32 * PQ_EPP * 2);
   const int tid = threadIdx.x, lane = tid & 63, wave = __builtin_amdgcn_readfirstlane(tid >> 6), r = lane & 31, h = lane >> 5;
   d16* stg = stg_all + wave * (32 * PQ_EPP);
-  const int NT = a.N >> 5;
+  const int NT = KV ? (a.N >> 5) / 3 * 2 : a.N >> 5;
   const int mw = blockIdx.x * (32 * NW) + wave * 32;
   const int m = mw + r, mc = m < a.M ? m : a.M - 1;
 
   auto issue = [&](int t) {
     constexpr int PW = 32 / NW;
-    const d16* src = a.Wf + (long long)t * PQ_TILE_ELEMS + wave * (PW * 512) + lane * 8;
+    const d16* src = a.Wf + (long long)pq_tile<KV>(t) * PQ_TILE_ELEMS + wave * (PW * 512) + lane * 8;
     d16* dst = ring + (t & 1) * PQ_TILE_ELEMS + wave * (PW * 512);
     __builtin_amdgcn_global_load_lds((pq_gptr_t)src, (pq_lptr_t)dst, 16, 0, 0);
     __builtin_amdgcn_global_load_lds((pq_gptr_t)src, (pq_lptr_t)dst, 16, 1024, 0);
@@ -208,8 +210,8 @@
   }
   const unsigned ring_l = (unsigned)reinterpret_cast<uintptr_t>(ring) + lane * 16;
 
-  auto store_block = [&](int u) {
-    const int head = u / 3, part = u - head * 3;
+  auto store_block = [&](int j) {
+    const int u = pq_block<KV>(j), head = u / 3, part = u - head * 3;
     d16* cbase = (part == 1 ? a.Kc : a.Vc) + (long long)head * a.max_ctx * 64;
 #pragma unroll
     for (int it = 0; it < 4; ++it) {
@@ -250,10 +252,11 @@
     PQ_RD4(wf[0], 0);                                                                                                    \
     PQ_GROUP(c, 0); PQ_GROUP(c, 1); PQ_GROUP(c, 2); PQ_GROUP(c, 3); PQ_GROUP(c, 4); PQ_GROUP(c, 5); PQ_GROUP(c, 6); PQ_GROUP(c, 7); \
   } while (0)
-  for (int u = 0; u < (NT >> 1); ++u) {
+  for (int j = 0; j < (NT >> 1); ++j) {
+    const int u = pq_block<KV>(j);
     f32x16 c0, c1;
-    PQ_TILE(c0, 2 * u);
-    PQ_TILE(c1, 2 * u + 1);
+    PQ_TILE(c0, 2 * j);
+    PQ_TILE(c1, 2 * j + 1);
     asm volatile("s_nop 15\n\ts_nop 15" : "+v"(c1) : : "memory");
     {
       const int part = u % 3;
@@ -284,14 +287,18 @@
 }
 
 int launch_pqkv(const PQkvArgs& a, hipStream_t st) {
-  if (a.M <= 0 || a.N != 1536 || a.ldx < 512 || (a.ldx % 8) || !a.X || !a.Wf || !a.bias || !a.Qb || !a.Kc || !a.Vc || !a.rows.pos || !a.rows.slot || !a.rows.active ||
+  if (a.M <= 0 || a.N != 1536 || a.ldx < 512 || (a.ldx % 8) || !a.X || !a.Wf || !a.bias || (!a.Qb && !a.kv_only) || !a.Kc || !a.Vc || !a.rows.pos || !a.rows.slot || !a.rows.active ||
       !a.rope_cos || !a.rope_sin || a.n_heads != 8 || (((uintptr_t)a.X | (uintptr_t)a.Wf | (uintptr_t)a.Qb | (uintptr_t)a.Kc | (uintptr_t)a.Vc) & 15) || (a.slot_stride % 8))
     ETD_FAIL(ETD_EINVAL, "pqkv: bad arguments");
   ETD_LAUNCH_FILTER("k_pqkv");
-  ProfScope ps("k_pqkv", st, 2.0 * a.M * a.N * 512.0, ((double)a.M * 512 + (double)a.N * 512 + 3.0 * a.M * 512) * 2);
+  const double nfrac = a.kv_only ? 2.0 / 3.0 : 1.0;
+  ProfScope ps("k_pqkv", st, 2.0 * a.M * a.N * nfrac * 512.0, ((double)a.M * 512 + (double)a.N * nfrac * 512 + 3.0 * nfrac * a.M * 512) * 2);
   static const int nw = getenv("ETD_PQKV_WAVES") ? atoi(getenv("ETD_PQKV_WAVES")) : 8;
-  if (nw == 4) hipLaunchKernelGGL(k_pqkv<4>, dim3((a.M + 127) / 128), dim3(256), 0, st, a);
-  else hipLaunchKernelGGL(k_pqkv<8>, dim3((a.M + 255) / 256), dim3(512), 0, st, a);
+  if (a.kv_only) {
+    if (nw == 4) hipLaunchKernelGGL((k_pqkv<4, true>), dim3((a.M + 127) / 128), dim3(256), 0, st, a);
+    else hipLaunchKernelGGL((k_pqkv<8, true>), dim3((a.M + 255) / 256), dim3(512), 0, st, a);
+  } else if (nw == 4) hipLaunchKernelGGL((k_pqkv<4, false>), dim3((a.M + 127) / 128), dim3(256), 0, st, a);
+  else hipLaunchKernelGGL((k_pqkv<8, false>), dim3((a.M + 255) / 256), dim3(512), 0, st, a);
   HIP_TRY(hipGetLastError());
   return ETD_OK;
 }
diff --git a/include/etude_hip_debug.h b/include/etude_hip_debug.h
--- a/include/etude_hip_debug.h
+++ b/include/etude_hip_debug.h
@@ -28,6 +28,9 @@
 int etd_debug_decoder_trace_lanes(etd_dec*, float* out_host, long long cap_floats, int n_active, void* stream);
 int etd_debug_decoder_trace_q(etd_dec*, float* out_host, long long cap_floats, int n_active, void* stream);
 int etd_debug_decoder_peek_kv(etd_dec*, int layer, int slot, int head, int n_pos, unsigned short* k_out, unsigned short* v_out, void* stream);
+int etd_debug_decoder_peek(etd_dec*, int what, int layer, int pos0, int n_pos, void* out_host, long long cap_bytes, void* stream);
+int etd_debug_resid_ln_rows(const float* P, int k_splits, const float* bias, const float* add, const float* hin, float* hout, int M, int H, const float* g1,
+                            const float* b1, const float* g2, const float* b2, float eps, void* x1, void* x2, void* stream);
 int etd_debug_decoder_trace_read(etd_dec*, unsigned* out_host, long long cap_words, int n_active, int* steps_done, void* stream);
 
 int etd_debug_decoder_force_pair(etd_dec*, int mode);
```

After: 590.2, median of 2. No clear change (+0.3%).
